# saghen/frizbee

Hardware: AMD Instinct MI355X
Metric: haystacks scored/sec (whole node) + achieved HBM GB/s, 6-char needle vs 10M len-32 haystacks (higher is better)
Workload: dtype u8; 1 GPU; needle 'deadbe' (6 chars) vs 10,000,000 x 32-byte ASCII haystacks per GPU, max_typos=0, mix 5% full / 20% partial / 75% none, seed 12345 (BASELINE.json configs[1]); haystacks_per_gpu=10000000, haystack_len=32, max_typos=0, emulated_reference_backend=AVX-512 (prefilter 64 lanes, Smith-Waterman 64 x u8), ranks_seen=1, backend=none (single process), filter_survivors=499537

## Files before the change

### frizbee_amd/__init__.py

```python
import ctypes as C
import weakref
import enum
import os
from copy import deepcopy
from dataclasses import dataclass, field, replace

import numpy as np

_HERE = os.path.dirname(os.path.abspath(__file__))
_LIB_PATH = os.environ.get("FRIZBEE_HIP_LIB", os.path.join(_HERE, "libfrizbee_hip.so"))

MATCH_DTYPE = np.dtype([("index", "<u4"), ("score", "<u2"), ("exact", "u1"), ("_pad", "u1")])
MATCH_INDICES_DTYPE = np.dtype([("index", "<u4"), ("score", "<u2"), ("exact", "u1"), ("_pad", "u1"), ("positions_begin", "<u4"), ("positions_len", "<u4")])


class FrizbeeError(RuntimeError):
    def __init__(self, code, msg):
        super().__init__(msg)
        self.code = code


class PanicError(FrizbeeError):
    """The reference would `panic!` here; the message is the reference's panic text."""

# ... 47 lines not shown
    max_typos: "int | None" = 0
    casing: CaseMatching = CaseMatching.Smart
    unicode: UnicodeMatching = UnicodeMatching.Smart
    sort: SortStrategy = SortStrategy.ScoreThenIndexAsc
    scoring: Scoring = field(default_factory=Scoring)
    pf_lanes: int = 0
    sw_lanes: int = 0
    matching: Matching = Matching.Fuzzy


class _CScoring(C.Structure):
    _fields_ = [(n, C.c_uint16) for n in ("match_score", "mismatch_penalty", "gap_open_penalty", "gap_extend_penalty", "prefix_bonus",
                                          "capitalization_bonus", "matching_case_bonus", "exact_match_bonus", "delimiter_bonus")]


class _CConfig(C.Structure):
    _fields_ = [("max_typos", C.c_int32), ("casing", C.c_int32), ("unicode", C.c_int32), ("sort", C.c_int32), ("scoring", _CScoring),
                ("pf_lanes", C.c_uint16), ("sw_lanes", C.c_uint16), ("matching", C.c_int32)]


class _CPattern(C.Structure):
    _fields_ = [("needle_utf8", C.c_void_p), ("needle_len", C.c_size_t), ("negated", C.c_int32), ("has_max_typos", C.c_int32), ("max_typos", C.c_int32),
                ("casing", C.c_int32), ("unicode", C.c_int32), ("has_scoring", C.c_int32), ("scoring", _CScoring), ("matching", C.c_int32)]


_lib = None

SYMBOLS = [
    "fzb_last_error", "fzb_config_default", "fzb_matcher_create", "fzb_matcher_clone", "fzb_matcher_free", "fzb_matcher_info", "fzb_matcher_set_pattern", "fzb_matcher_set_config",
    "fzb_corpus_upload", "fzb_corpus_from_device", "fzb_corpus_set_max_len", "fzb_corpus_set_uniform_len", "fzb_corpus_free", "fzb_corpus_len", "fzb_match_list", "fzb_match_list_into",
    "fzb_match_list_device", "fzb_match_list_sorted_device", "fzb_match_list_parallel", "fzb_matches_free", "fzb_radix_sort_matches", "fzb_k_merge_matches",
    "fzb_matcher_reserve", "fzb_debug_unicode_dfa_accepts", "fzb_set_profiling", "fzb_last_timings", "fzb_last_stage_timings", "fzb_last_counters",
    "fzb_multi_matcher_create", "fzb_multi_matcher_free", "fzb_multi_matcher_len", "fzb_multi_match_list", "fzb_multi_match_list_device",
    "fzb_parse_query", "fzb_patterns_free", "fzb_match_list_indices", "fzb_match_indices_free", "fzb_multi_match_list_indices",
    "fzb_match_list_indices_into", "fzb_multi_match_list_into", "fzb_multi_match_list_indices_into",
    "fzb_device_count", "fzb_shard_ranges", "fzb_corpus_upload_sharded", "fzb_sharded_corpus_free", "fzb_sharded_corpus_len", "fzb_sharded_corpus_shards",
    "fzb_sharded_corpus_shard", "fzb_match_list_parallel_sharded", "fzb_debug_lcs_dfa_accepts", "fzb_debug_cdfa_state",
    "fzb_merge_shard_runs", "fzb_corpus_build_view", "fzb_debug_reload_knobs", "fzb_matcher_shard_report",
    "fzb_rccl_unique_id", "fzb_shard_comm_create", "fzb_shard_comm_free", "fzb_shard_comm_rank", "fzb_shard_comm_world", "fzb_match_list_parallel_rccl",
    "fzb_shard_comm_last_exchange",
    "fzb_multi_matcher_set_patterns", "fzb_multi_matcher_set_config", "fzb_multi_matcher_reserve", "fzb_multi_matcher_clone", "fzb_multi_match_list_parallel",
    "fzb_multi_match_list_parallel_sharded", "fzb_multi_match_list_parallel_rccl", "fzb_multi_matcher_shard_report", "fzb_debug_device_allocs",
    "fzb_match_list_top", "fzb_match_list_top_device", "fzb_multi_match_list_top", "fzb_match_list_top_sharded", "fzb_multi_match_list_top_sharded",
    "fzb_corpus_reserve", "fzb_corpus_append", "fzb_corpus_truncate", "fzb_corpus_info", "fzb_debug_corpus_read",
    "fzb_corpus_remove", "fzb_corpus_remove_device", "fzb_corpus_replace", "fzb_corpus_edit_info",
    "fzb_match_list_top_indices", "fzb_match_list_top_indices_device", "fzb_matcher_reserve_top_indices", "fzb_multi_match_list_top_indices",
    "fzb_multi_match_list_top_indices_device", "fzb_multi_match_list_top_indices_fused", "fzb_multi_matcher_reserve_top_indices",
    "fzb_corpus_signature_info", "fzb_debug_needle_signature", "fzb_debug_signature_threshold", "fzb_debug_set_filter_grid",
    "fzb_corpus_set_bias", "fzb_corpus_update_bias", "fzb_corpus_clear_bias", "fzb_corpus_bias_info",
    "fzb_corpus_set_tags", "fzb_corpus_update_tags", "fzb_corpus_clear_tags", "fzb_corpus_set_scope", "fzb_corpus_scope_info",
    "fzb_corpus_generation", "fzb_subset_create", "fzb_subset_free", "fzb_subset_set_indices", "fzb_subset_from_scope", "fzb_subset_info", "fzb_subset_read",
    "fzb_match_list_subset", "fzb_match_list_top_subset", "fzb_match_list_top_subset_device", "fzb_match_list_top_indices_subset",
    "fzb_multi_match_list_subset", "fzb_multi_match_list_top_subset", "fzb_multi_match_list_top_subset_device", "fzb_multi_match_list_top_indices_subset",
    "fzb_debug_set_items_dfa_min", "fzb_debug_set_fused_capture", "fzb_debug_launch_grids", "fzb_corpus_signature_planes_info",
    "fzb_prompt_list_device", "fzb_prompt_top_device",
    "fzb_facets_create", "fzb_facets_free", "fzb_facets_read", "fzb_facets_device", "fzb_matcher_set_facets", "fzb_multi_matcher_set_facets",
    "fzb_match_list_top_sections", "fzb_match_list_top_sections_device", "fzb_multi_match_list_top_sections", "fzb_multi_match_list_top_sections_device",
]


def lib():
    global _lib
    if _lib is None:
        if not os.path.exists(_LIB_PATH):
            raise FrizbeeError(4, f"{_LIB_PATH} is missing: build it with `python -c 'import __graft_entry__ as g; g.build()'` (make -C frizbee_amd/csrc)")
        l = C.CDLL(_LIB_PATH)
        l.fzb_last_error.restype = C.c_char_p
        l.fzb_config_default.argtypes = [C.POINTER(_CConfig)]
        l.fzb_matcher_create.argtypes = [C.POINTER(_CConfig), C.c_char_p, C.c_size_t, C.POINTER(C.c_void_p)]
        l.fzb_matcher_clone.argtypes = [C.c_void_p, C.POINTER(C.c_void_p)]
        l.fzb_matcher_free.argtypes = [C.c_void_p]
        l.fzb_matcher_set_pattern.argtypes = [C.c_void_p, C.c_char_p, C.c_size_t]
        l.fzb_matcher_set_config.argtypes = [C.c_void_p, C.POINTER(_CConfig)]
        l.fzb_matcher_info.argtypes = [C.c_void_p, C.POINTER(C.c_int32)]
        l.fzb_corpus_upload.argtypes = [C.c_void_p, C.c_void_p, C.c_size_t, C.POINTER(C.c_void_p)]
        l.fzb_corpus_from_device.argtypes = [C.c_void_p, C.c_void_p, C.c_int, C.c_size_t, C.c_uint64, C.POINTER(C.c_void_p)]
        l.fzb_corpus_set_max_len.argtypes = [C.c_void_p, C.c_uint32]
        l.fzb_corpus_set_uniform_len.argtypes = [C.c_void_p, C.c_uint32]
        l.fzb_corpus_free.argtypes = [C.c_void_p]
        l.fzb_corpus_len.argtypes = [C.c_void_p]
        l.fzb_corpus_len.restype = C.c_size_t
        l.fzb_match_list.argtypes = [C.c_void_p, C.c_void_p, C.POINTER(C.c_void_p), C.POINTER(C.c_size_t)]
        l.fzb_match_list_into.argtypes = [C.c_void_p, C.c_void_p, C.c_size_t, C.c_size_t, C.c_uint32, C.POINTER(C.c_void_p), C.POINTER(C.c_size_t)]
        l.fzb_match_list_device.argtypes = [C.c_void_p, C.c_void_p, C.c_size_t, C.c_size_t, C.c_uint32, C.c_void_p, C.c_size_t, C.c_void_p, C.c_void_p]
        l.fzb_match_list_sorted_device.argtypes = [C.c_void_p, C.c_void_p, C.c_void_p, C.c_size_t, C.c_void_p, C.c_void_p]
        l.fzb_match_list_parallel.argtypes = [C.c_void_p, C.c_void_p, C.c_size_t, C.POINTER(C.c_void_p), C.POINTER(C.c_size_t)]
        l.fzb_matches_free.argtypes = [C.c_void_p]
        l.fzb_radix_sort_matches.argtypes = [C.c_void_p, C.c_size_t]
        l.fzb_k_merge_matches.argtypes = [C.c_int32, C.c_void_p, C.c_void_p, C.c_size_t, C.c_void_p]
        l.fzb_matcher_reserve.argtypes = [C.c_void_p, C.c_void_p]
        l.fzb_debug_unicode_dfa_accepts.argtypes = [C.c_void_p, C.c_char_p, C.c_size_t]
        l.fzb_set_profiling.argtypes = [C.c_void_p, C.c_int]
        l.fzb_last_timings.argtypes = [C.c_void_p, C.POINTER(C.c_float)]
        l.fzb_last_stage_timings.argtypes = [C.c_void_p, C.POINTER(C.c_float)]
        l.fzb_last_counters.argtypes = [C.c_void_p, C.POINTER(C.c_uint32)]
        l.fzb_multi_matcher_create.argtypes = [C.POINTER(_CConfig), C.POINTER(_CPattern), C.c_size_t, C.POINTER(C.c_void_p)]
        l.fzb_multi_matcher_free.argtypes = [C.c_void_p]
        l.fzb_parse_query.argtypes = [C.c_char_p, C.c_size_t, C.POINTER(C.POINTER(_CPattern)), C.POINTER(C.c_size_t)]
        l.fzb_patterns_free.argtypes = [C.POINTER(_CPattern), C.c_size_t]
        l.fzb_multi_matcher_len.argtypes = [C.c_void_p]
        l.fzb_multi_matcher_len.restype = C.c_size_t
        l.fzb_multi_match_list.argtypes = [C.c_void_p, C.c_void_p, C.POINTER(C.c_void_p), C.POINTER(C.c_size_t)]
        l.fzb_multi_match_list_device.argtypes = [C.c_void_p, C.c_void_p, C.c_size_t, C.c_size_t, C.c_uint32, C.c_void_p, C.c_size_t, C.c_void_p, C.c_void_p]
        l.fzb_match_list_indices.argtypes = [C.c_void_p, C.c_void_p, C.c_void_p, C.c_size_t, C.POINTER(C.c_void_p), C.POINTER(C.c_size_t), C.POINTER(C.c_void_p)]
        l.fzb_match_indices_free.argtypes = [C.c_void_p, C.c_void_p]
        l.fzb_multi_match_list_indices.argtypes = l.fzb_match_list_indices.argtypes
        l.fzb_match_list_indices_into.argtypes = [C.c_void_p, C.c_void_p, C.c_void_p, C.c_size_t, C.c_uint32, C.POINTER(C.c_void_p), C.POINTER(C.c_size_t), C.POINTER(C.c_void_p)]
# ... 4 lines not shown
        l.fzb_corpus_upload_sharded.argtypes = [C.c_void_p, C.c_void_p, C.c_size_t, C.c_int, C.c_int, C.POINTER(C.c_void_p)]
        l.fzb_sharded_corpus_free.argtypes = [C.c_void_p]
        l.fzb_sharded_corpus_len.argtypes = [C.c_void_p]
        l.fzb_sharded_corpus_len.restype = C.c_size_t
        l.fzb_sharded_corpus_shards.argtypes = [C.c_void_p]
        l.fzb_sharded_corpus_shard.argtypes = [C.c_void_p, C.c_int, C.POINTER(C.c_uint64), C.POINTER(C.c_uint64), C.POINTER(C.c_int)]
        l.fzb_match_list_parallel_sharded.argtypes = [C.c_void_p, C.c_void_p, C.POINTER(C.c_void_p), C.POINTER(C.c_size_t)]
        l.fzb_matcher_shard_report.argtypes = [C.c_void_p]
        l.fzb_matcher_shard_report.restype = C.c_char_p
        l.fzb_merge_shard_runs.argtypes = [C.c_void_p, C.c_void_p, C.c_void_p, C.c_void_p, C.c_size_t, C.c_void_p, C.POINTER(C.c_void_p), C.POINTER(C.c_size_t)]
        l.fzb_corpus_build_view.argtypes = [C.c_void_p, C.POINTER(C.c_int)]
        l.fzb_rccl_unique_id.argtypes = [C.c_void_p]
        l.fzb_shard_comm_create.argtypes = [C.c_void_p, C.c_int, C.c_int, C.POINTER(C.c_void_p)]
        l.fzb_shard_comm_free.argtypes = [C.c_void_p]
        l.fzb_shard_comm_rank.argtypes = [C.c_void_p]
        l.fzb_shard_comm_world.argtypes = [C.c_void_p]
        l.fzb_match_list_parallel_rccl.argtypes = [C.c_void_p, C.c_void_p, C.c_uint32, C.c_void_p, C.c_int, C.POINTER(C.c_void_p), C.POINTER(C.c_size_t)]
        l.fzb_shard_comm_last_exchange.argtypes = [C.c_void_p, C.POINTER(C.c_uint64)]
        l.fzb_debug_lcs_dfa_accepts.argtypes = [C.c_void_p, C.c_char_p, C.c_size_t, C.POINTER(C.c_int32)]
        l.fzb_debug_cdfa_state.argtypes = [C.c_void_p, C.c_char_p, C.c_size_t, C.POINTER(C.c_int32)]
        l.fzb_multi_matcher_set_patterns.argtypes = [C.c_void_p, C.POINTER(_CPattern), C.c_size_t]
        l.fzb_multi_matcher_set_config.argtypes = [C.c_void_p, C.POINTER(_CConfig)]
        l.fzb_multi_matcher_reserve.argtypes = [C.c_void_p, C.c_void_p]
        l.fzb_multi_matcher_clone.argtypes = [C.c_void_p, C.POINTER(C.c_void_p)]
        l.fzb_multi_match_list_parallel.argtypes = l.fzb_match_list_parallel.argtypes
        l.fzb_multi_match_list_parallel_sharded.argtypes = l.fzb_match_list_parallel_sharded.argtypes
        l.fzb_multi_match_list_parallel_rccl.argtypes = l.fzb_match_list_parallel_rccl.argtypes
        l.fzb_multi_matcher_shard_report.argtypes = [C.c_void_p]
        l.fzb_multi_matcher_shard_report.restype = C.c_char_p
        l.fzb_debug_device_allocs.argtypes = [C.POINTER(C.c_uint64)]
        l.fzb_match_list_top.argtypes = [C.c_void_p, C.c_void_p, C.c_size_t, C.POINTER(C.c_void_p), C.POINTER(C.c_size_t), C.POINTER(C.c_uint64)]
        l.fzb_match_list_top_device.argtypes = [C.c_void_p, C.c_void_p, C.c_size_t, C.c_void_p, C.c_size_t, C.c_void_p, C.c_void_p]
        l.fzb_multi_match_list_top.argtypes = l.fzb_match_list_top.argtypes
        l.fzb_match_list_top_sharded.argtypes = l.fzb_match_list_top.argtypes
        l.fzb_multi_match_list_top_sharded.argtypes = l.fzb_match_list_top.argtypes
        l.fzb_corpus_reserve.argtypes = [C.c_void_p, C.c_size_t, C.c_uint64]
        l.fzb_corpus_append.argtypes = [C.c_void_p, C.c_void_p, C.c_void_p, C.c_size_t]
        l.fzb_corpus_truncate.argtypes = [C.c_void_p, C.c_size_t]
        l.fzb_corpus_info.argtypes = [C.c_void_p, C.POINTER(C.c_uint64)]
        l.fzb_debug_corpus_read.argtypes = [C.c_void_p, C.c_int, C.c_void_p, C.c_size_t, C.POINTER(C.c_size_t)]
        l.fzb_corpus_remove.argtypes = [C.c_void_p, C.c_void_p, C.c_size_t]
        l.fzb_corpus_remove_device.argtypes = [C.c_void_p, C.c_void_p, C.c_size_t, C.c_void_p, C.c_size_t]
        l.fzb_corpus_replace.argtypes = [C.c_void_p, C.c_void_p, C.c_size_t, C.c_void_p, C.c_void_p]
        l.fzb_corpus_edit_info.argtypes = [C.c_void_p, C.POINTER(C.c_uint64)]
        l.fzb_match_list_top_indices.argtypes = [C.c_void_p, C.c_void_p, C.c_size_t, C.POINTER(C.c_void_p), C.POINTER(C.c_size_t), C.POINTER(C.c_void_p), C.POINTER(C.c_uint64)]
        l.fzb_match_list_top_indices_device.argtypes = [C.c_void_p, C.c_void_p, C.c_size_t, C.c_void_p, C.c_size_t, C.c_void_p, C.c_size_t, C.c_void_p, C.c_void_p]
        l.fzb_matcher_reserve_top_indices.argtypes = [C.c_void_p, C.c_void_p, C.c_size_t, C.c_size_t]
        l.fzb_multi_match_list_top_indices.argtypes = l.fzb_match_list_top_indices.argtypes
        l.fzb_multi_match_list_top_indices_fused.argtypes = l.fzb_match_list_top_indices.argtypes
        l.fzb_multi_match_list_top_indices_device.argtypes = l.fzb_match_list_top_indices_device.argtypes
        l.fzb_multi_matcher_reserve_top_indices.argtypes = l.fzb_matcher_reserve_top_indices.argtypes
        l.fzb_corpus_signature_info.argtypes = [C.c_void_p, C.POINTER(C.c_int), C.POINTER(C.c_uint64)]
        l.fzb_corpus_signature_planes_info.argtypes = l.fzb_corpus_signature_info.argtypes
        l.fzb_debug_needle_signature.argtypes = [C.c_void_p, C.POINTER(C.c_uint32), C.POINTER(C.c_int)]
        l.fzb_debug_signature_threshold.argtypes = []
        l.fzb_debug_signature_threshold.restype = C.c_uint32
        l.fzb_debug_set_filter_grid.argtypes = [C.c_int]
        l.fzb_debug_set_filter_grid.restype = None
        l.fzb_corpus_set_bias.argtypes = [C.c_void_p, C.c_void_p, C.c_size_t]
        l.fzb_corpus_update_bias.argtypes = [C.c_void_p, C.c_void_p, C.c_void_p, C.c_size_t]
        l.fzb_corpus_clear_bias.argtypes = [C.c_void_p]
        l.fzb_corpus_bias_info.argtypes = [C.c_void_p, C.POINTER(C.c_uint64)]
        l.fzb_corpus_set_tags.argtypes = [C.c_void_p, C.c_void_p, C.c_size_t]
        l.fzb_corpus_update_tags.argtypes = [C.c_void_p, C.c_void_p, C.c_void_p, C.c_size_t]
        l.fzb_corpus_clear_tags.argtypes = [C.c_void_p]
        l.fzb_corpus_set_scope.argtypes = [C.c_void_p, C.c_uint16, C.c_uint16]
        l.fzb_corpus_scope_info.argtypes = [C.c_void_p, C.POINTER(C.c_uint64)]
        l.fzb_debug_set_items_dfa_min.argtypes = [C.c_uint32]
        l.fzb_debug_set_items_dfa_min.restype = None
        l.fzb_debug_set_fused_capture.argtypes = [C.c_int]
        l.fzb_debug_set_fused_capture.restype = None
        l.fzb_debug_launch_grids.argtypes = [C.c_char_p, C.c_size_t, C.POINTER(C.c_size_t), C.c_int]
        l.fzb_corpus_generation.argtypes = [C.c_void_p, C.POINTER(C.c_uint64)]
        l.fzb_subset_create.argtypes = [C.c_void_p, C.POINTER(C.c_void_p)]
        l.fzb_subset_free.argtypes = [C.c_void_p]
        l.fzb_subset_free.restype = None
        l.fzb_subset_set_indices.argtypes = [C.c_void_p, C.c_void_p, C.c_size_t]
        l.fzb_subset_from_scope.argtypes = [C.c_void_p, C.c_void_p, C.c_uint16, C.c_uint16]
        l.fzb_subset_info.argtypes = [C.c_void_p, C.POINTER(C.c_uint64)]
        l.fzb_subset_read.argtypes = [C.c_void_p, C.c_void_p, C.c_size_t, C.POINTER(C.c_size_t)]
        l.fzb_match_list_subset.argtypes = [C.c_void_p, C.c_void_p, C.c_void_p, C.c_void_p, C.POINTER(C.c_void_p), C.POINTER(C.c_size_t)]
        l.fzb_match_list_top_subset.argtypes = [C.c_void_p, C.c_void_p, C.c_void_p, C.c_void_p, C.c_size_t, C.POINTER(C.c_void_p), C.POINTER(C.c_size_t), C.POINTER(C.c_uint64)]
        l.fzb_match_list_top_subset_device.argtypes = [C.c_void_p, C.c_void_p, C.c_void_p, C.c_void_p, C.c_size_t, C.c_void_p, C.c_size_t, C.c_void_p, C.c_void_p]
        l.fzb_multi_match_list_subset.argtypes = l.fzb_match_list_subset.argtypes
        l.fzb_multi_match_list_top_subset.argtypes = l.fzb_match_list_top_subset.argtypes
        l.fzb_multi_match_list_top_subset_device.argtypes = l.fzb_match_list_top_subset_device.argtypes
        l.fzb_prompt_list_device.argtypes = [C.c_void_p, C.c_void_p, C.c_void_p, C.c_size_t, C.c_size_t, C.c_uint32, C.c_void_p, C.c_size_t, C.c_void_p, C.c_void_p]
        l.fzb_prompt_top_device.argtypes = [C.c_void_p, C.c_void_p, C.c_void_p, C.c_size_t, C.c_void_p, C.c_size_t, C.c_void_p, C.c_void_p]
        l.fzb_match_list_top_indices_subset.argtypes = [C.c_void_p, C.c_void_p, C.c_void_p, C.c_void_p, C.c_size_t, C.POINTER(C.c_void_p), C.POINTER(C.c_size_t), C.POINTER(C.c_void_p),
                                                        C.POINTER(C.c_uint64)]
        l.fzb_multi_match_list_top_indices_subset.argtypes = l.fzb_match_list_top_indices_subset.argtypes
        l.fzb_facets_create.argtypes = [C.c_void_p, C.POINTER(C.c_void_p)]
        l.fzb_facets_free.argtypes = [C.c_void_p]
        l.fzb_facets_free.restype = None
        l.fzb_facets_read.argtypes = [C.c_void_p, C.POINTER(C.c_uint32)]
        l.fzb_facets_device.argtypes = [C.c_void_p]
        l.fzb_facets_device.restype = C.c_void_p
        l.fzb_matcher_set_facets.argtypes = [C.c_void_p, C.c_void_p]
        l.fzb_multi_matcher_set_facets.argtypes = [C.c_void_p, C.c_void_p]
        l.fzb_match_list_top_sections.argtypes = [C.c_void_p, C.c_void_p, C.c_void_p, C.c_size_t, C.c_size_t, C.c_void_p, C.c_void_p, C.POINTER(C.c_void_p), C.POINTER(C.c_size_t),
                                                  C.POINTER(C.c_uint64)]
        l.fzb_match_list_top_sections_device.argtypes = [C.c_void_p, C.c_void_p, C.c_void_p, C.c_size_t, C.c_size_t, C.c_void_p, C.c_void_p, C.c_void_p, C.c_size_t, C.c_void_p, C.c_void_p]
        l.fzb_multi_match_list_top_sections.argtypes = l.fzb_match_list_top_sections.argtypes
        l.fzb_multi_match_list_top_sections_device.argtypes = l.fzb_match_list_top_sections_device.argtypes
        _lib = l
    return _lib
# ... 85 lines not shown
        self.h = C.c_void_p()
        self._keep = keep
        _check(lib().fzb_corpus_from_device(dev_bytes_ptr, dev_ends_ptr, int(ends_are_u64), n, total_bytes, C.byref(self.h)))
        if uniform_len:
            _check(lib().fzb_corpus_set_uniform_len(self.h, uniform_len))
        if max_len:
            _check(lib().fzb_corpus_set_max_len(self.h, max_len))
        return self

    def build_view(self):
        built = C.c_int()
        _check(lib().fzb_corpus_build_view(self.h, C.byref(built)))
        return bool(built.value)

    def append(self, haystacks=None, *, packed=None):
        data, ends = packed if packed is not None else pack(haystacks)
        data = np.ascontiguousarray(data, dtype=np.uint8)
        ends = np.ascontiguousarray(ends, dtype=np.uint64)
        _check(lib().fzb_corpus_append(self.h, data.ctypes.data, ends.ctypes.data if len(ends) else None, len(ends)))

    def reserve(self, items, nbytes):
        _check(lib().fzb_corpus_reserve(self.h, items, nbytes))

    def truncate(self, n):
        _check(lib().fzb_corpus_truncate(self.h, n))

    def remove(self, indices):
        ix = np.ascontiguousarray(indices, dtype=np.uint32)
        _check(lib().fzb_corpus_remove(self.h, ix.ctypes.data if len(ix) else None, len(ix)))

    def remove_device(self, ptr, stride, count_ptr, max_count):
        _check(lib().fzb_corpus_remove_device(self.h, ptr, stride, count_ptr, max_count))

    def replace(self, indices, haystacks=None, *, packed=None):
        ix = np.ascontiguousarray(indices, dtype=np.uint32)
        data, ends = packed if packed is not None else pack(haystacks)
        data = np.ascontiguousarray(data, dtype=np.uint8)
        ends = np.ascontiguousarray(ends, dtype=np.uint64)
        if len(ix) != len(ends):
            raise FrizbeeError(1, f"Corpus.replace: {len(ix)} indices for {len(ends)} haystacks")
        _check(lib().fzb_corpus_replace(self.h, ix.ctypes.data if len(ix) else None, len(ix), data.ctypes.data, ends.ctypes.data if len(ends) else None))

    EDIT_INFO_FIELDS = ("first", "bytes_written", "view_tiles", "temp_bytes")

    def edit_info(self):
        out = (C.c_uint64 * 4)()
        _check(lib().fzb_corpus_edit_info(self.h, out))
        return dict(zip(self.EDIT_INFO_FIELDS, (int(v) for v in out)))

    INFO_FIELDS = ("items", "item_capacity", "bytes", "byte_capacity", "max_len", "uniform_len", "has_view", "view_nv", "outliers", "ends_u64", "regrows",
                   "h2d_bytes")
    DEBUG_ARRAYS = {"bytes": (0, np.uint8), "ends": (1, None), "vbytes": (2, np.uint8), "vgofs": (3, np.uint32), "vgnv": (4, np.uint8), "vlen": (5, np.uint16),
                    "vperm": (6, np.uint16), "vlong": (7, np.uint32), "sig": (8, np.uint32), "bias": (9, np.int16), "tags": (10, np.uint16),
                    "sig_planes": (11, np.uint64)}

    def set_bias(self, values):
        if values is None:
            _check(lib().fzb_corpus_clear_bias(self.h))
            return
        v = np.asarray(values)
        if v.size and (v.min() < -32768 or v.max() > 32767):
            raise FrizbeeError(1, "Corpus.set_bias: a bias is a signed 16-bit value")
        v = np.ascontiguousarray(v, dtype=np.int16)
        _check(lib().fzb_corpus_set_bias(self.h, v.ctypes.data if len(v) else None, len(v)))

    def _update_column(self, fn, who, indices, v):
        ix = np.ascontiguousarray(indices, dtype=np.uint32)
        if len(ix) != len(v):
            raise FrizbeeError(1, f"{who}: {len(ix)} indices for {len(v)} values")
        _check(fn(self.h, ix.ctypes.data if len(ix) else None, v.ctypes.data if len(v) else None, len(ix)))

    def update_bias(self, indices, values):
        v = np.asarray(values)
        if v.size and (v.min() < -32768 or v.max() > 32767):
            raise FrizbeeError(1, "Corpus.update_bias: a bias is a signed 16-bit value")
        self._update_column(lib().fzb_corpus_update_bias, "Corpus.update_bias", indices, np.ascontiguousarray(v, dtype=np.int16))

    BIAS_INFO_FIELDS = ("has_bias", "capacity", "bias_hi", "device_bytes")

    def bias_info(self):
        out = (C.c_uint64 * 4)()
        _check(lib().fzb_corpus_bias_info(self.h, out))
        return dict(zip(self.BIAS_INFO_FIELDS, (int(x) for x in out)))

    @staticmethod
    def _tags16(values, who):
        v = np.asarray(values)
        if v.size and (v.dtype.kind not in "iub" or v.min() < 0 or v.max() > 65535):
            raise FrizbeeError(1, f"{who}: tags are 16 caller-defined bits (0 .. 65535)")
        return np.ascontiguousarray(v, dtype=np.uint16)

    def set_tags(self, values):
        v = self._tags16(values, "Corpus.set_tags")
        _check(lib().fzb_corpus_set_tags(self.h, v.ctypes.data if len(v) else None, len(v)))

    def update_tags(self, indices, values):
        ix = np.asarray(indices)
        if ix.size and (ix.min() < 0 or ix.max() > 0xFFFFFFFF):
            raise FrizbeeError(1, "Corpus.update_tags: an index is an unsigned 32-bit value")
        self._update_column(lib().fzb_corpus_update_tags, "Corpus.update_tags", ix, self._tags16(values, "Corpus.update_tags"))

    def clear_tags(self):
        _check(lib().fzb_corpus_clear_tags(self.h))

    def set_scope(self, require=0, exclude=0):
        for name, v in (("require", require), ("exclude", exclude)):
            if not 0 <= int(v) <= 65535:
                raise FrizbeeError(1, f"Corpus.set_scope: {name} is a 16-bit mask (0 .. 65535)")
        _check(lib().fzb_corpus_set_scope(self.h, int(require), int(exclude)))

    SCOPE_INFO_FIELDS = ("active", "capacity", "scope", "device_bytes")

    def scope_info(self):
        out = (C.c_uint64 * 4)()
        _check(lib().fzb_corpus_scope_info(self.h, out))
        d = dict(zip(self.SCOPE_INFO_FIELDS, (int(x) for x in out)))
        d["require"], d["exclude"] = d["scope"] & 0xFFFF, d["scope"] >> 16
        return d

    def signature_info(self):
        built, nbytes = C.c_int(), C.c_uint64()
        _check(lib().fzb_corpus_signature_info(self.h, C.byref(built), C.byref(nbytes)))
        return bool(built.value), int(nbytes.value)

    def signature_planes_info(self):
        built, nbytes = C.c_int(), C.c_uint64()
        _check(lib().fzb_corpus_signature_planes_info(self.h, C.byref(built), C.byref(nbytes)))
        return bool(built.value), int(nbytes.value)

    def info(self):
        out = (C.c_uint64 * 12)()
        _check(lib().fzb_corpus_info(self.h, out))
        return dict(zip(self.INFO_FIELDS, (int(v) for v in out)))

    def debug_read(self, what):
        code, dtype = self.DEBUG_ARRAYS[what]
        if dtype is None:
            dtype = np.uint64 if self.info()["ends_u64"] else np.uint32
        n = C.c_size_t()
        rc = lib().fzb_debug_corpus_read(self.h, code, None, 0, C.byref(n))
        if rc != 5:
            _check(rc)
        buf = np.zeros(n.value, np.uint8)
        if n.value:
            _check(lib().fzb_debug_corpus_read(self.h, code, buf.ctypes.data, buf.nbytes, C.byref(n)))
        return buf.view(dtype)

    def generation(self):
        out = C.c_uint64()
        _check(lib().fzb_corpus_generation(self.h, C.byref(out)))
        return out.value

    def __len__(self):
        return lib().fzb_corpus_len(self.h)

    def __del__(self):
        try:
            if getattr(self, "h", None):
                lib().fzb_corpus_free(self.h)
                self.h = None
        except Exception:
            pass


SHARD_BY_COUNT, SHARD_BY_BYTES, SHARD_OVERSUBSCRIBE = 0, 1, 2


class Subset:

    def __init__(self, corpus):
        self.corpus = corpus
        self.h = C.c_void_p()
        _check(lib().fzb_subset_create(corpus.h, C.byref(self.h)))

    def set_indices(self, indices):
        a = np.asarray(indices)
        if a.size and (a.dtype.kind not in "iu" or int(a.min()) < 0 or int(a.max()) > 0xFFFFFFFF):
            raise ValueError("Subset.set_indices: the indices must be integers that fit uint32")
        a = np.ascontiguousarray(a, dtype=np.uint32)
        _check(lib().fzb_subset_set_indices(self.h, a.ctypes.data if len(a) else None, len(a)))
# ... 688 lines not shown
```

### frizbee_amd/csrc/fzb_internal.h

```cpp
#pragma once
#include <stddef.h>
#include <stdint.h>

typedef uint8_t u8;
typedef uint16_t u16;
typedef uint32_t u32;
typedef uint64_t u64;

#define FZB_MAX_ROWS 63
#define FZB_MAX_NEEDLE_BYTES 64
#define FZB_MAX_HAYSTACK_LEN 1024
#define FZB_UNICODE_FWD_CAP 4096u
#define FZB_TILE 1024

struct NeedleDev {
    int32_t rows;
    int32_t nbytes;
    int32_t max_typos;
    int32_t min_haystack_len;
    int32_t unicode;
    int32_t lane_mask;
    u16 match_plus_mismatch;
    u16 mismatch;
    u16 gex;
    u16 gopm;
    u16 prefix, capitalization, matching_case, exact_bonus, delimiter;
    u16 match_score, gap_open;
    u16 _pad;
    alignas(4) u8 raw[FZB_MAX_NEEDLE_BYTES];
    alignas(4) u8 c[FZB_MAX_NEEDLE_BYTES];
    alignas(4) u8 f[FZB_MAX_NEEDLE_BYTES];
    u8 uc[FZB_MAX_ROWS + 1][4];
    u8 uf[FZB_MAX_ROWS + 1][4];
    u8 ulen[FZB_MAX_ROWS + 1];
    static constexpr bool kLong = false;
};

struct NeedleLongDev {
    int32_t rows, nbytes, max_typos, min_haystack_len, unicode, lane_mask;
    u16 match_plus_mismatch, mismatch, gex, gopm;
    u16 prefix, capitalization, matching_case, exact_bonus, delimiter;
    u16 match_score, gap_open, _pad;
    const u8* raw;
    const u8* c;
    const u8* f;
    const u8 (*uc)[4];
    const u8 (*uf)[4];
    const u8* ulen;
    static constexpr bool kLong = true;
};

struct CorpusDev {
    const u8* bytes;
    const void* ends;
    u64 n;
    u64 total_bytes;
    int ends_u64;
    u32 max_len;
    u32 uniform_len;
    const u8* vbytes;
    const u32* vgofs;
    const u8* vgnv;
    const u16* vlen;
    const u16* vperm;
    u32 view_nv;
    const u32* vlong;
    u32 n_long;
    const u32* sig;
    const u64* sig_planes;
};

struct fzb_match_rec {
    u32 index;
    u16 score;
    u8 exact;
    u8 valid;
};

struct fzb_indices_rec {
    u32 index;
    u16 score;
    u8 exact;
    u8 _pad;
    u32 positions_begin;
    u32 positions_len;
};

struct SortBuffers {
    fzb_match_rec* tmp;
    u32* hist;
    size_t cap;
};

struct Workspace {
    u64* bitmap;
    u32* tile_counts;
    u32* surv_idx;
    u32* win;
    u32* overflow;
    u32* dp_scratch;
    size_t dp_scratch_words;
    SortBuffers sort;
    u64* bitmap2;
    u32* tile_counts2;
    u32* items2;
    u32* win2;
    u32* seg_counts;
    u32* counters;
    u64* bitmap_m;
    u32* tile_counts_m;
    u32* marg_list;
    u64* reject_bits;
    u32* tile_rejects;
    u32* rej_prefix;
    size_t cap_marg;
    u32* cls_win;
    u32* cls_lists;
    size_t cap_cls;
    u64* table;
    u8* dfa;
    u8* uni_dfa;
    u8* lcs_dfa;
// ... 1 lines not shown
    size_t cap_items;
    size_t cap_level2;
    bool tables_stale;
    u8* tables_blob;
    u8* tables_host;
    hipEvent_t tables_ev;
    bool tables_ev_pending;
    u32* trace_cells;
    size_t trace_cells_words;
};

struct LaunchCfg {
    int pf_lanes, sw_lanes;
    int filter_mode;
    int filter_exact;
    int window_mode;
    int bias_ok;
    int pad_ok;
    int cfu_ok;
    int cf_ok;
    int cfm_ok;
    int num_cus;
    u32 dead_byte;
};

#define FZB_MAX_RUNS 64
struct RunSet {
    const fzb_match_rec* run[FZB_MAX_RUNS];
    const u32* count[FZB_MAX_RUNS];
    u32 cap[FZB_MAX_RUNS];
    int n;
};

struct RejectOut {
    u64* bits;
    u32* tile_rejects;
    u32* rej_prefix;
    u32* count;
};

struct SegList {
    u32* list;
    u32* counts;
    u32 nseg, stride;
    u32* total_out;
};

#ifdef __HIPCC__
#include <hip/hip_runtime.h>
void fzb_launch_filter(const CorpusDev& c, u64 first, u32 count, const u64* table, const u8* dfa, u32 dead, int rows, int mode, int need, u32 min_len,
                       u64* bitmap, u32* tile_counts, u32* reset_counters, int grid, hipStream_t st, u64* bitmap_m = nullptr, u32* tile_counts_m = nullptr,
                       u64* reject_bits = nullptr, u32* tile_rejects = nullptr, int nul_safe = 0, int acc_lo = -1, const u8* cdfa = nullptr, u32 cdfa_bytes = 0,
                       int cdfa_K = 0, int cdfa_G = 0, u32 needle_sig = 0, int sig_ok = 0,
                       const SegList* seg = nullptr);
bool fzb_filter_sig_applies(const CorpusDev& c, int mode, u32 needle_sig, int sig_ok);
void fzb_launch_sig_planes(const u32* sig, u64 n, u64 t0, u64* planes, int grid, hipStream_t st);
void fzb_launch_scan_rejects(const u32* tile_rejects, u32 ntiles, const u32* reject_count, u32* rej_prefix, hipStream_t st);
void fzb_launch_init_counters(u32* counters, u32 n0, hipStream_t st);
void fzb_launch_compact1(const u64* bitmap, const u32* counts, u32 n_items, const u32* n_items_ptr, const u32* src, u32* out_idx, u32* total_out, int grid, hipStream_t st,
                         u32* total_out2 = nullptr);
void fzb_launch_filter_items(const CorpusDev& c, u64 first, const u32* items, const u32* n_items_ptr, const u64* table, int rows, int mode, int need, u32 min_len,
                             u64* bitmap, u32* tile_counts, int grid, hipStream_t st, const u8* dfa = nullptr, int exact = 0, u32 needle_sig = 0, int sig_ok = 0, u64 n_hint = 0);
bool fzb_filter_items_dfa_applies(const CorpusDev& c, int mode, int exact, const u8* dfa, int rows, u64 n_hint);
void fzb_launch_compact2(const u64* bitmap, const u32* counts, const u32* n_items_ptr, const u32* in_idx, const u32* in_win, u32* out_idx, u32* out_win, u32* total_out,
                         int grid, hipStream_t st);
void fzb_launch_window(const CorpusDev& c, u64 first, const u32* surv_idx, const u32* n_surv_ptr, const NeedleDev& nd, int pf_lanes,
                       u32* win, u64* bitmap2, u32* tile_counts2, u32* counters, int grid, hipStream_t st, const RejectOut* decide = nullptr, u32 max_items = 0);
void fzb_launch_dp(const CorpusDev& c, u64 first, u32 index_offset, const u32* items, const u32* win, const u32* n_items_ptr, const NeedleDev& nd,
                   int sw_lanes, int mode, int wmode, int pad_ok, fzb_match_rec* out, u32 capacity, u32* dev_count, u32* overflow, u32 qcap, u32* counters, int grid, hipStream_t st,
                   const RejectOut* rejects = nullptr, const SegList* seg = nullptr);
bool fzb_dp_short_applies(const CorpusDev& c, int sw_lanes, int mode);
void fzb_launch_compact1_classify(const CorpusDev& c, u64 first, const u64* bitmap, const u32* tile_counts, u32 n_items, u32* out_idx, u32* total_out, const NeedleDev& nd, int sw_lanes,
                                  int wmode, u32 capacity, u32* dev_count, u32* overflow, u32 qcap, u32* counters, u32* win_out, u32* lists, u32 list_stride, int grid, hipStream_t st,
                                  int split_multi);
void fzb_launch_dp_classes(const CorpusDev& c, u64 first, u32 index_offset, const u32* items, const u32* win_in, const u32* n_items_ptr, const NeedleDev& nd, int sw_lanes,
                           int wmode, fzb_match_rec* out, u32 capacity, u32* dev_count, u32* overflow, u32 qcap, u32* counters, u32* win_out, u32* lists, u32 list_stride,
                           int num_cus, hipStream_t st, int part = 0, int split_multi = 0);
void fzb_launch_classes_all(const CorpusDev& c, u64 first, u32 index_offset, const u32* items, const u32* win, const u32* lists, u32 list_stride, const u32* counters,
                            const NeedleDev& nd, int sw_lanes, fzb_match_rec* out, u32 capacity, u32* scratch, int gm, int gc, hipStream_t st);
void fzb_launch_dp_multi(const CorpusDev& c, u64 first, u32 index_offset, const u32* list, const u32* n_list_ptr, const NeedleDev& nd, int sw_lanes, int mode,
                         fzb_match_rec* out, u32 capacity, u32* scratch, int grid, hipStream_t st);
void fzb_launch_unicode_split_wide(const CorpusDev& c, u64 first, const u32* items, const u32* n_items_ptr, int sw_lanes, u32 capacity, u32* overflow, u32 qcap, u32* counters,
                                   int grid, hipStream_t st);
void fzb_launch_dp_unicode(const CorpusDev& c, u64 first, u32 index_offset, const u32* items, const u32* win, const u32* n_items_ptr, const NeedleDev& nd,
                           int sw_lanes, int wmode, fzb_match_rec* out, u32 capacity, u32* dev_count, u32* overflow, u32 qcap, u32* counters,
                           int grid, hipStream_t st, int tform = 0, int multi_front = 0, int one_round_wgs = 0);
void fzb_launch_dp_unicode_multi(const CorpusDev& c, u64 first, u32 index_offset, const u32* list, const u32* n_list_ptr, const NeedleDev& nd, int sw_lanes,
                                 fzb_match_rec* out, u32 capacity, u32* scratch, int grid, hipStream_t st, u32 only_from = 0, int tform = 0, u32* counters = nullptr,
                                 u32* back_end = nullptr, u32 fwd_cap = 0);
void fzb_launch_sort(fzb_match_rec* buf, fzb_match_rec* tmp, const u32* n_ptr, u32* hist, u32 ntiles_cap, int reverse_first, int by_score, int grid, hipStream_t st, int passes = 2);
void fzb_launch_concat_runs(const RunSet& rs, const u32* base_in, u32* total_out, fzb_match_rec* out, u32 capacity, int grid, u32* cut_flag, hipStream_t st);
hipError_t fzb_launch_topk_select(const fzb_match_rec* in, const u32* in_count, u32 in_cap, u32 limit, int by_score, int desc, int one_pass, fzb_match_rec* out, u32 out_cap,
                            u32* out_count, u32* scratch, u32 ntiles_cap, int grid, hipStream_t st);
void fzb_launch_topk_concat(const RunSet& rs, const u32* base_in, u32* total_out, fzb_match_rec* out, u32 capacity, int grid, hipStream_t st);
struct sections_set;
size_t fzb_sections_scratch_words(size_t n_records);
hipError_t fzb_launch_sections_select(const fzb_match_rec* in, const u32* in_count, u32 in_cap, const uint16_t* tags, u64 n_tags, const sections_set& ss, u32 limit, int by_score,
                                      int desc, int one_pass, fzb_match_rec* out, u32* counts, u32* scratch, u32 ntiles_cap, int grid, hipStream_t st);
void fzb_launch_bias_apply(fzb_match_rec* recs, const u32* count, u32 cap, const int16_t* bias, u64 n_bias, u64 first, u32 index_offset, int grid_max, hipStream_t st);
void fzb_launch_scope_drop(const fzb_match_rec* recs, const u32* count, u32 cap, const uint16_t* tags, u64 n_tags, u64 first, u32 index_offset, u32 require, u32 exclude, u64* bitmap,
                           u32* tile_counts, fzb_match_rec* out, u32 capacity, u32* count_out, int grid_max, hipStream_t st, u32* facets = nullptr);
void fzb_launch_facets_records(const fzb_match_rec* recs, const u32* count, u32 cap, const uint16_t* tags, u64 n_tags, u64 first, u32 index_offset, u32 require, u32 exclude, u32* block,
                               int grid_max, hipStream_t st);
void fzb_launch_facets_column(const u32* items, const u32* n_ptr, u32 n, u32 hint, const uint16_t* tags, u64 n_tags, u64 first, u32 require, u32 exclude, u32* block, int grid_max,
                              hipStream_t st);
void fzb_launch_top_items(const fzb_match_rec* head, const u32* head_count, u32 cap, u32* items, u32* n_items, u32* dev_count, int grid, hipStream_t st);
size_t fzb_indices_pack_tile_words(size_t max_records);
void fzb_launch_indices_pack(const fzb_match_rec* head, const u32* head_count, const fzb_match_rec* traced, const u32* traced_count, const u32* npos, const u32* pos, u32 stride,
                             fzb_indices_rec* out, u32 out_cap, u32* dense, u32 dense_cap, u32* dev_count, u32* tiles, u32 max_records, int grid, hipStream_t st);
// ... 49 lines not shown
```

### frizbee_amd/csrc/host.hip

```cpp
#include <hip/hip_runtime.h>

#include <algorithm>
#include <chrono>
#include <cstdio>
#include <cstdlib>
#include <cstring>
#include <memory>
#include <mutex>
#include <new>
#include <thread>
#include <string>
#include <map>
#include <unordered_map>
#include <vector>

#include "host_internal.h"
#include "sig_filter.h"
#include "score_bias.h"
#include "scope.h"
#include "sections.h"
#include "seg_list.h"

namespace {
#include "unicode_case_table.inc"
// ... 740 lines not shown
    m->needle.assign((const char*)needle_utf8, needle_len);
    m->empty = needle_len == 0;
    const fzb_scoring& sc = config->scoring;
    m->use_u8 = fits_in_u8(needle_len, sc);
    int pf = config->pf_lanes, sw = config->sw_lanes;
    if (pf == 0 && sw == 0) detect_host_lanes(m->use_u8, pf, sw);
    else if (sw == 0) sw = m->use_u8 ? pf : pf / 2;
    if (!(pf == 16 || pf == 32 || pf == 64) || !(sw == 8 || sw == 16 || sw == 32 || sw == 64))
        return fail(FZB_ERR_INVALID, "pf_lanes must be 16/32/64 and sw_lanes 8/16/32/64 (or both 0 = auto)");
    m->lc.pf_lanes = pf;
    m->lc.sw_lanes = sw;
    if (m->empty) return FZB_OK;
    bool any_upper = false, ascii = true;
    for (u32 cp : cps) { any_upper |= is_uppercase(cp); ascii &= cp < 0x80; }
    m->case_sensitive = config->casing == FZB_CASE_RESPECT || (config->casing == FZB_CASE_SMART && any_upper);
    m->unicode = config->unicode == FZB_UNICODE_ALWAYS || (config->unicode == FZB_UNICODE_SMART && !ascii);
    m->rows = (int)(m->unicode ? cps.size() : needle_len);
    if (config->matching < FZB_MATCH_FUZZY || config->matching > FZB_MATCH_SUBSTRING) return fail(FZB_ERR_INVALID, "bad matching mode");
    m->literal_mode = config->matching;
    std::string perr = m->literal_mode ? overflow_guard(sc, needle_len, sadd16(std::max(sc.capitalization_bonus, sc.delimiter_bonus), sc.matching_case_bonus), 0)
                                       : overflow_guard(sc, (size_t)m->rows);
    if (!perr.empty()) return fail(FZB_ERR_PANIC, perr);
    m->long_needle = needle_len > FZB_MAX_NEEDLE_BYTES || m->rows > FZB_MAX_ROWS;
    fill_needle_scalars(m, needle_len, cps.size());
    if (m->long_needle) {
        build_long_needle(m, needle_utf8, needle_len, cps);
        return FZB_OK;
    }
    NeedleDev& nd = m->nd;
    for (size_t i = 0; i < needle_len; i++) {
        nd.raw[i] = nd.c[i] = needle_utf8[i];
        nd.f[i] = flip_ascii_byte(m, needle_utf8[i]);
    }
    for (size_t i = 0; i < cps.size() && cps.size() <= FZB_MAX_ROWS; i++) {
        nd.ulen[i] = (u8)encode_utf8(cps[i], nd.uc[i]);
        encode_utf8(m->case_sensitive ? cps[i] : flip_same_width(cps[i]), nd.uf[i]);
    }
    const int k = config->max_typos;
    LaunchCfg& lc = m->lc;
    if (k < 0 || k >= m->rows) {
        lc.filter_mode = 0; lc.filter_exact = 1; lc.window_mode = 2;
    } else if (!m->unicode && k == 0) {
        lc.filter_mode = 1; lc.filter_exact = 1; lc.window_mode = 1;
    } else {
        lc.filter_mode = k == 0 ? 1 : 2; lc.filter_exact = 0; lc.window_mode = 0;
    }
    build_filter_tables(m);
    build_unicode_dfa(m);
    build_lcs_dfa(m);
    build_cdfa(m);
    set_scorer_forms(m, needle_utf8, needle_len);
    m->sig_eligible = !m->unicode && lc.filter_mode == 1 && lc.filter_exact && needle_sig_eligible(needle_utf8, needle_len, k, m->literal_mode);
    m->needle_sig = m->sig_eligible ? needle_sig(needle_utf8, needle_len) : 0u;
    return FZB_OK;
}

int fzb_matcher_create(const fzb_config* config, const uint8_t* needle_utf8, size_t needle_len, fzb_matcher** out) {
    if (!out) return fail(FZB_ERR_INVALID, "null argument");
    std::unique_ptr<fzb_matcher> mp(new fzb_matcher());
    if (int rc = compile_needle(*mp, config, needle_utf8, needle_len)) return rc;
    *out = mp.release();
    return FZB_OK;
}

static int rebuild_matcher(fzb_matcher* m, const fzb_config* config, const uint8_t* needle_utf8, size_t needle_len) {
    CompiledNeedle fresh;
    int rc = compile_needle(fresh, config, needle_utf8, needle_len);
    if (rc) return rc;
    const int num_cus = m->lc.num_cus;
    static_cast<CompiledNeedle&>(*m) = std::move(fresh);
    m->lc.num_cus = num_cus;
    m->ws.tables_stale = true;
    if (m->long_blob_dev) (void)hipFree(m->long_blob_dev);
    m->long_blob_dev = nullptr;
    memset(m->last_counters, 0, sizeof(m->last_counters));
    if (!m->shard_clones.empty()) {
        fzb_config ccfg = m->config;
        ccfg.pf_lanes = (uint16_t)m->lc.pf_lanes;
        ccfg.sw_lanes = (uint16_t)m->lc.sw_lanes;
        bool ok = true;
        for (fzb_matcher* cm : m->shard_clones) ok = ok && rebuild_matcher(cm, &ccfg, needle_utf8, needle_len) == FZB_OK;
        if (!ok) {
            std::vector<fzb_matcher*> drop;
            drop.swap(m->shard_clones);
            for (fzb_matcher* cm : drop) fzb_matcher_free(cm);
            fzb_clear_error();
        }
    }
    return FZB_OK;
}

int fzb_matcher_set_pattern(fzb_matcher* m, const uint8_t* needle_utf8, size_t needle_len) {
    if (!m || (!needle_utf8 && needle_len)) return fail(FZB_ERR_INVALID, "null argument");
    if (m->needle.size() == needle_len && (needle_len == 0 || memcmp(m->needle.data(), needle_utf8, needle_len) == 0)) return FZB_OK;
    const fzb_config cfg = m->config;
    return rebuild_matcher(m, &cfg, needle_utf8, needle_len);
}

}
static bool same_scoring(const fzb_scoring& a, const fzb_scoring& b) {
    return a.match_score == b.match_score && a.mismatch_penalty == b.mismatch_penalty && a.gap_open_penalty == b.gap_open_penalty && a.gap_extend_penalty == b.gap_extend_penalty &&
           a.prefix_bonus == b.prefix_bonus && a.capitalization_bonus == b.capitalization_bonus && a.matching_case_bonus == b.matching_case_bonus &&
           a.exact_match_bonus == b.exact_match_bonus && a.delimiter_bonus == b.delimiter_bonus;
}
static bool same_config(const fzb_config& a, const fzb_config& b) {
    return a.max_typos == b.max_typos && a.casing == b.casing && a.unicode == b.unicode && a.sort == b.sort && a.pf_lanes == b.pf_lanes && a.sw_lanes == b.sw_lanes &&
// ... 65 lines not shown
    if (!fzb_knobs().verify_promises || !c->dev.n || (!uniform_len && !max_len)) return FZB_OK;
    unsigned long long* d = nullptr;
    int prev_dev = 0, own_dev = 0;
    HIPCHK(hipGetDevice(&prev_dev));
    own_dev = prev_dev;
    hipPointerAttribute_t attr;
    if (hipPointerGetAttributes(&attr, c->dev.ends) == hipSuccess && attr.type == hipMemoryTypeDevice) own_dev = attr.device;
    else (void)hipGetLastError();
    struct DeviceGuard {
        int prev, cur;
        ~DeviceGuard() { if (cur != prev) (void)hipSetDevice(prev); }
    } guard{prev_dev, own_dev};
    if (own_dev != prev_dev) HIPCHK(hipSetDevice(own_dev));
    HIPCHK(hipDeviceSynchronize());
    HIPCHK(dev_alloc((void**)&d, 16));
    const unsigned long long init[2] = {0ull, ~0ull};
    hipError_t e = hipMemcpy(d, init, 16, hipMemcpyHostToDevice);
    if (e == hipSuccess) {
        const int grid = (int)fzb_grid_cap((c->dev.n + 255) / 256, 16);
        if (c->dev.ends_u64) FZB_LAUNCH((k_verify_promise<u64>), dim3(grid), dim3(256), 0, 0, (const u64*)c->dev.ends, c->dev.n, c->dev.total_bytes, uniform_len, max_len, d);
        else FZB_LAUNCH((k_verify_promise<u32>), dim3(grid), dim3(256), 0, 0, (const u32*)c->dev.ends, c->dev.n, c->dev.total_bytes, uniform_len, max_len, d);
        e = hipGetLastError();
    }
    unsigned long long got[2] = {0, 0};
    if (e == hipSuccess) e = hipMemcpy(got, d, 16, hipMemcpyDeviceToHost);
    (void)hipFree(d);
    if (e != hipSuccess) return fail(FZB_ERR_HIP, std::string("verifying the corpus promise: ") + hipGetErrorString(e));
    if (got[0])
        return fail(FZB_ERR_INVALID, std::string(what) + ": the end offsets contradict it for " + std::to_string(got[0]) + " haystack(s), first at index " + std::to_string(got[1]) +
                                         " (checked on the device; FZB_VERIFY_PROMISES=0 skips the check)");
    return FZB_OK;
}
extern "C" {
int fzb_corpus_from_device(const void* dev_bytes, const void* dev_ends, int ends_are_u64, size_t n, uint64_t total_bytes, fzb_corpus** out) {
    if (!out || (n && (!dev_bytes || !dev_ends))) return fail(FZB_ERR_INVALID, "null argument");
    if (((uintptr_t)dev_bytes & 15) != 0) return fail(FZB_ERR_INVALID, "dev_bytes must be 16-byte aligned");
    if (n > 0xFFFFFFFFull) return fail(FZB_ERR_PANIC, "too many items in haystack, will overflow the u32 index: " + std::to_string(n) + " > 4294967295 (index offset: 0)");
    auto c = new fzb_corpus();
    c->dev.bytes = (const u8*)dev_bytes;
    c->dev.ends = dev_ends;
    c->dev.ends_u64 = ends_are_u64 != 0;
    c->dev.n = n;
    c->dev.total_bytes = total_bytes;
    *out = c;
    return FZB_OK;
}

void fzb_corpus_free(fzb_corpus* c) {
    if (!c) return;
    if (c->own_bytes) (void)hipFree(c->own_bytes);
    if (c->own_ends) (void)hipFree(c->own_ends);
    if (c->own_sig) (void)hipFree(c->own_sig);
    if (c->own_planes) (void)hipFree(c->own_planes);
    fzb_column_release(c->bias);
    fzb_column_release(c->tags);
    if (c->pair_stage) (void)hipFree(c->pair_stage);
    for (void* q : c->own_view)
        if (q) (void)hipFree(q);
    for (void* q : {c->stage_raw, c->stage_ends, c->stage_tiles, c->stage_stats})
        if (q) (void)hipFree(q);
    delete c;
}
size_t fzb_corpus_len(const fzb_corpus* c) { return c ? (size_t)c->dev.n : 0; }
int fzb_corpus_set_uniform_len(fzb_corpus* c, uint32_t len) {
    if (!c) return fail(FZB_ERR_INVALID, "null argument");
    if (c->own_bytes) {
        if (len == c->dev.uniform_len) return FZB_OK;
        return fail(FZB_ERR_INVALID, "the corpus was uploaded by fzb_corpus_upload, which detected its lengths itself (uniform length " + std::to_string(c->dev.uniform_len) +
                                         ", 0 = not uniform); the promise can only be made for borrowed device memory");
    }
    if (len && (u64)((len + 15u) & ~15u) * (c->dev.n ? c->dev.n - 1 : 0) + len > c->dev.total_bytes) return fail(FZB_ERR_INVALID, "uniform length does not fit the corpus buffer");
    if (len) {
        const int vrc = verify_promise(c, len, 0, ("a uniform length of " + std::to_string(len) + " bytes was promised").c_str());
        if (vrc) return vrc;
    }
    if (!len && c->dev.uniform_len && c->dev.max_len == c->dev.uniform_len) c->dev.max_len = 0;
    c->dev.uniform_len = len;
    if (len) c->dev.max_len = len;
    return fzb_sig_sync_borrowed(c);
}

int fzb_corpus_set_max_len(fzb_corpus* c, uint32_t max_len) {
    if (!c) return fail(FZB_ERR_INVALID, "null argument");
    if (c->own_bytes) {
        if (max_len == 0 || max_len >= c->dev.max_len) return FZB_OK;
        return fail(FZB_ERR_INVALID, "the corpus was uploaded by fzb_corpus_upload, which measured its longest haystack (" + std::to_string(c->dev.max_len) + " bytes); " +
                                         std::to_string(max_len) + " is not an upper bound");
    }
    if (c->dev.uniform_len) {
        if (max_len == 0 || max_len >= c->dev.uniform_len) return FZB_OK;
        return fail(FZB_ERR_INVALID, "the corpus promises a uniform length of " + std::to_string(c->dev.uniform_len) + " bytes; " + std::to_string(max_len) + " is not an upper bound");
    }
    if (max_len && max_len != c->dev.uniform_len) {
        const int vrc = verify_promise(c, 0, max_len, ("a longest haystack of " + std::to_string(max_len) + " bytes was promised").c_str());
        if (vrc) return vrc;
    }
    c->dev.max_len = max_len;
    return fzb_sig_sync_borrowed(c);
}

}
int fzb_bind_device(fzb_matcher* m) {
    int dev = 0;
    HIPCHK(hipGetDevice(&dev));
    if (m->device >= 0) {
        if (dev != m->device)
// ... 527 lines not shown
static int g_debug_filter_grid = 0;
static bool pipe_seg_applies(const Pipe& p) {
    const fzb_matcher* m = p.m;
    const LaunchCfg& lc = m->lc;
    return !p.items_in && !p.trace && !fzb_knobs().no_seg_list && !m->nd.unicode && m->sig_eligible && lc.filter_mode == 1 && lc.filter_exact && lc.window_mode == 1 && lc.cf_ok &&
           fzb_filter_sig_applies(p.cd, 1, m->needle_sig, 1) && fzb_dp_short_applies(p.cd, lc.sw_lanes, 2);
}
static int pipe_filter_stage(Pipe& p) {
    fzb_matcher* m = p.m;
    Workspace& w = m->ws;
    const LaunchCfg& lc = m->lc;
    const NeedleDev& nd = m->nd;
    u32* cnt_c = w.counters;
    p.n_items_ptr = &cnt_c[0];
    p.wmode = lc.window_mode;
    const int need = nd.rows - (nd.max_typos > 0 ? nd.max_typos : 0);
    int exact_wmode = 0;
    const bool uni_typo_exact = nd.unicode && lc.filter_mode == 2 && m->lcs_scalar && m->lcs_states && lc.bias_ok && !p.trace && !fzb_knobs().typo_exact_window && p.cd.max_len != 0 &&
                                p.cd.max_len <= (u32)lc.pf_lanes;
    if (p.items_in) {
        if (lc.filter_mode == 0) {
            HIPCHK(hipMemcpyAsync(&cnt_c[0], p.n_items_in, 4, hipMemcpyDeviceToDevice, p.st));
            p.items = p.items_in;
        } else {
            fzb_launch_filter_items(p.cd, p.first, p.items_in, p.n_items_in, w.table, nd.rows, lc.filter_mode, need, (u32)nd.min_haystack_len, w.bitmap, w.tile_counts, p.cus * 4, p.st,
                                    nd.unicode ? nullptr : w.dfa, lc.filter_exact, m->needle_sig, m->sig_eligible, p.items_hint);
            FZB_STAGE("filter(items)");
            fzb_launch_compact1(w.bitmap, w.tile_counts, 0, p.n_items_in, p.items_in, w.surv_idx, &cnt_c[0], p.cus * 2, p.st);
            FZB_STAGE("compact1(items)");
            p.items = w.surv_idx;
        }
    } else if (lc.filter_mode == 0) {
    } else if (m->uni_dfa_states && lc.bias_ok && !p.trace) {
        FZB_PEV(2);
        fzb_launch_filter(p.cd, p.first, p.cnt, w.table, w.uni_dfa, lc.dead_byte, m->uni_dfa_states - 1, 1, 0, (u32)nd.min_haystack_len, w.bitmap, w.tile_counts, w.counters, p.cus * 8, p.st, nullptr,
                          nullptr, nullptr, nullptr, lc.pad_ok, -1, m->cdfa_src == 2 ? w.cdfa : nullptr, (u32)m->cdfa.size(), m->cdfa_K, m->cdfa_G);
        FZB_PEV(3);
        FZB_STAGE("filter(unicode dfa)");
        fzb_launch_compact1(w.bitmap, w.tile_counts, p.cnt, nullptr, nullptr, w.surv_idx, &cnt_c[0], p.cus * 4, p.st, &cnt_c[1]);
        FZB_STAGE("compact1");
        p.items = w.surv_idx;
        exact_wmode = 1;
    } else if (pipe_seg_applies(p)) {
        const u32 ntiles = (p.cnt + FZB_TILE - 1) / FZB_TILE;
        u32 grid = std::min<u32>(std::min<u32>((u32)p.cus * 8u, FZB_SEG_MAX), ntiles);
        if (g_debug_filter_grid > 0) grid = std::min<u32>(grid, (u32)g_debug_filter_grid);
        grid = std::max<u32>(grid, 1u);
        const u32 stride = tc_tiles_per_run(ntiles, grid) * FZB_TILE;
        if ((size_t)ntiles * FZB_TILE > w.cap_items) return fail(FZB_ERR_INVALID, "internal: the survivor list does not hold the range rounded up to a tile");
        p.seg = SegList{w.surv_idx, w.seg_counts, grid, stride, &cnt_c[0]};
        p.segmented = true;
        FZB_PEV(2);
        fzb_launch_filter(p.cd, p.first, p.cnt, w.table, w.dfa, lc.dead_byte, nd.rows, 1, need, (u32)nd.min_haystack_len, w.bitmap, w.tile_counts, w.counters, (int)grid, p.st, nullptr, nullptr,
                          nullptr, nullptr, lc.pad_ok, -1, nullptr, 0, 0, 0, m->needle_sig, 1, &p.seg);
        FZB_PEV(3);
        FZB_STAGE("filter(lists its survivors)");
        p.items = w.surv_idx;
    } else {
        FZB_PEV(2);
        if (lc.filter_mode == 2 && m->lcs_states)
            fzb_launch_filter(p.cd, p.first, p.cnt, w.table, w.lcs_dfa, lc.dead_byte, m->lcs_states - 1, 1, need, (u32)nd.min_haystack_len, w.bitmap, w.tile_counts, w.counters, p.cus * 8, p.st, nullptr,
                              nullptr, nullptr, nullptr, lc.pad_ok, m->lcs_acc_lo, m->cdfa_src == 3 ? w.cdfa : nullptr, (u32)m->cdfa.size(), m->cdfa_K, m->cdfa_G);
        else
            fzb_launch_filter(p.cd, p.first, p.cnt, w.table, w.dfa, lc.dead_byte, nd.rows, lc.filter_mode, need, (u32)nd.min_haystack_len, w.bitmap, w.tile_counts, w.counters, p.cus * 8, p.st, nullptr, nullptr,
                              nullptr, nullptr, lc.pad_ok, -1, (lc.filter_mode == 1 && m->cdfa_src == 1) ? w.cdfa : nullptr, (u32)m->cdfa.size(), m->cdfa_K, m->cdfa_G, m->needle_sig,
                              m->sig_eligible && lc.filter_mode == 1);
        FZB_PEV(3);
        FZB_STAGE("filter");
        const bool fuse = !nd.unicode && !p.trace && lc.filter_exact && !uni_typo_exact && (p.wmode == 1 || p.wmode == 2) && !fzb_knobs().no_fused_classify && w.cls_win && w.cls_lists &&
                          p.cnt <= (u32)p.cus * 2u * FZB_TILE && ascii_split_classes(m, p.cd);
        if (fuse) {
            fzb_launch_compact1_classify(p.cd, p.first, w.bitmap, w.tile_counts, p.cnt, w.surv_idx, &cnt_c[0], nd, lc.sw_lanes, p.wmode, p.cap32, p.dev_count, w.overflow, pipe_qcap(p), cnt_c,
                                         w.cls_win, w.cls_lists, (u32)w.cap_cls, p.cus * 4, p.st, 1);
            p.classified = true;
            FZB_STAGE("compact1 + classify");
        } else {
            fzb_launch_compact1(w.bitmap, w.tile_counts, p.cnt, nullptr, nullptr, w.surv_idx, &cnt_c[0], p.cus * 4, p.st, uni_typo_exact ? &cnt_c[1] : nullptr);
            FZB_STAGE("compact1");
        }
        p.items = w.surv_idx;
        if (uni_typo_exact) exact_wmode = 3;
    }
    if (exact_wmode) {
        p.wmode = exact_wmode;
    } else if (!lc.filter_exact) {
        fzb_launch_window(p.cd, p.first, p.items, &cnt_c[0], nd, lc.pf_lanes, w.win, w.bitmap2, w.tile_counts2, cnt_c, p.cus * 4, p.st, nullptr, p.items_in ? 0u : p.cnt);
        FZB_STAGE("window");
        fzb_launch_compact2(w.bitmap2, w.tile_counts2, &cnt_c[0], p.items, w.win, w.items2, w.win2, &cnt_c[1], p.cus * 2, p.st);
        FZB_STAGE("compact2");
        p.items = w.items2;
        p.win = w.win2;
        p.n_items_ptr = &cnt_c[1];
        p.wmode = 0;
    }
    return FZB_OK;
}

static bool ascii_split_classes(const fzb_matcher* m, const CorpusDev& cd) {
    const LaunchCfg& lc = m->lc;
    const FzbKnobs& kn = fzb_knobs();
    const bool no_wide = cd.max_len != 0 && cd.max_len <= (u32)lc.sw_lanes;
    const bool classes = lc.cf_ok && !kn.no_dp_classes && !fzb_dp_short_applies(cd, lc.sw_lanes, 2);
    return classes && !no_wide && lc.cfm_ok && !kn.no_dp_cfm;
}
static u32 pipe_qcap(const Pipe& p) { return (u32)std::min<u64>((u64)p.cnt + FZB_UNICODE_FWD_CAP, 0xFFFFFFFFull); }

static int traced_grid(int cus, size_t cnt) { return (int)std::max<size_t>(1, std::min<size_t>((size_t)cus / 2, (cnt + 3) / 4)); }
// ... 2545 lines not shown
```

### frizbee_amd/csrc/host_internal.h

```cpp
#pragma once
#include <hip/hip_runtime.h>

#include <array>
#include <atomic>
#include <functional>
#include <string>
#include <vector>

#include "../../include/frizbee_hip.h"
#include "fzb_internal.h"
#include "indices_union.h"
#include "knobs.h"

int fzb_fail(int code, const std::string& msg);
void fzb_clear_error();
#define HIPCHK(expr)                                                                                            \
    do {                                                                                                        \
        hipError_t e_ = (expr);                                                                                 \
        if (e_ != hipSuccess) return fzb_fail(FZB_ERR_HIP, std::string(#expr) + ": " + hipGetErrorString(e_)); \
    } while (0)

extern std::atomic<uint64_t> g_fzb_dev_allocs;
inline hipError_t fzb_dev_alloc(void** p, size_t bytes) {
    g_fzb_dev_allocs.fetch_add(1, std::memory_order_relaxed);
    return hipMalloc(p, bytes ? bytes : 16);
}

template <typename V>
struct ItemColumn {
    V* data = nullptr;
    u64 cap_items = 0;
    bool live = false;
};
template <typename V>
inline void fzb_column_release(ItemColumn<V>& col) {
    if (col.data) (void)hipFree(col.data);
    col = ItemColumn<V>{};
}

struct fzb_corpus {
    CorpusDev dev{};
    void* own_bytes = nullptr;
    void* own_ends = nullptr;
    void* own_view[6] = {nullptr, nullptr, nullptr, nullptr, nullptr, nullptr};
    u64 cap_items = 0;
    u64 cap_bytes = 0;
    u64 min_len = ~(u64)0;
    u64 max_len = 0;
    u64 n_over256 = 0;
    u64 max_short = 0;
    u64 view_units = 0;
    u64 view_items = 0;
    u64 view_cap_items = 0;
    u64 view_cap_units = 0;
    void* own_sig = nullptr;
    u64 sig_cap_items = 0;
    void* own_planes = nullptr;
    u64 planes_cap_tiles = 0;
    int sig_device = -1;
    ItemColumn<int16_t> bias;
    u32 bias_hi = 0;
    ItemColumn<uint16_t> tags;
    u32 scope_require = 0, scope_exclude = 0;
    void* pair_stage = nullptr;
    u64 pair_stage_cap = 0;
    u64 regrows = 0;
    u64 h2d_bytes = 0;
    u64 edit_info[4] = {0, 0, 0, 0};
    void* stage_raw = nullptr;
    void* stage_ends = nullptr;
    void* stage_tiles = nullptr;
    void* stage_stats = nullptr;
    u64 stage_raw_cap = 0, stage_items_cap = 0, stage_tiles_cap = 0;
    int device = -1;
    u64 generation = 0;
};
inline size_t fzb_corpus_reserved_items(const fzb_corpus* c) { return (size_t)(c->cap_items > c->dev.n ? c->cap_items : c->dev.n); }
inline const int16_t* fzb_corpus_bias(const fzb_corpus* c) { return c->bias.live ? c->bias.data : nullptr; }
inline u32 fzb_corpus_bias_hi(const fzb_corpus* c) { return c->bias.live ? c->bias_hi : 0; }
inline bool fzb_corpus_scoped(const fzb_corpus* c) { return c->tags.data && (c->scope_require | c->scope_exclude) != 0; }

struct fzb_subset {
    const fzb_corpus* corpus = nullptr;
    u64 generation = 0;
    u32* idx = nullptr;
    size_t cap = 0;
    u32* count_dev = nullptr;
    u64* bitmap = nullptr;
    u32* tiles = nullptr;
    bool known = true;
    u64 count = 0;
};

struct fzb_facets {
    const fzb_corpus* corpus = nullptr;
    u32* block = nullptr;
    u32* mirror = nullptr;
    hipEvent_t done = nullptr;
    bool on_event = false;
    bool pending = false;
    int device = -1;
};

template <typename T>
int fzb_dev_renew(T** p, size_t elems) {
    if (*p) HIPCHK(hipFree(*p));
    *p = nullptr;
    HIPCHK(fzb_dev_alloc((void**)p, elems * sizeof(T)));
    return FZB_OK;
}
template <typename T>
// ... 12 lines not shown
    u32* count_host = nullptr;
};
struct OutStaging {
    fzb_match_rec* out_dev = nullptr;
    size_t out_cap = 0;
    u32* count_dev = nullptr;
    FetchHint fetch;
    FetchHint fetch_top;
};
int fzb_out_ensure(OutStaging& o, size_t count);
void fzb_out_release(OutStaging& o);

struct ScopeScratch {
    fzb_match_rec* recs = nullptr;
    size_t recs_cap = 0;
    u64* bitmap = nullptr;
    size_t bitmap_words = 0;
    u32* tiles = nullptr;
    size_t tiles_cap = 0;
    u32* words = nullptr;
    size_t words_cap = 0;
};
int fzb_scope_ensure(ScopeScratch& s, size_t count);
int fzb_scope_ensure_flags(ScopeScratch& s, size_t count);
void fzb_scope_release(ScopeScratch& s);

struct SectionsScratch {
    u32* words = nullptr;
    size_t words_cap = 0;
    u32* stage = nullptr;
    size_t stage_words = 0;
};
int fzb_sections_ensure(SectionsScratch& s, size_t n_records, size_t stage_records);
void fzb_sections_release(SectionsScratch& s);

struct CompiledNeedle {
    fzb_config config{};
    std::string needle;
    bool empty = false, case_sensitive = false, unicode = false, use_u8 = false;
    int literal_mode = 0;
    int rows = 0;
    NeedleDev nd{};
    LaunchCfg lc{};
    std::vector<u64> table;
    std::vector<u8> dfa;
    std::vector<u8> uni_dfa;
    int uni_dfa_states = 0;
    std::vector<u8> lcs_dfa;
    int lcs_states = 0, lcs_acc_lo = 0;
    bool lcs_scalar = false;
    std::vector<u8> cdfa;
    int cdfa_src = 0, cdfa_K = 0, cdfa_G = 0;
    u32 needle_sig = 0;
    bool sig_eligible = false;
    bool long_needle = false;
    bool long_dfa = false;
    bool long_upper = false;
    NeedleLongDev ndl{};
    std::vector<u8> long_blob_host;
    size_t long_off_c = 0, long_off_f = 0, long_off_uc = 0, long_off_uf = 0, long_off_ulen = 0;
};

struct MatcherState : OutStaging {
    Workspace ws{};
    int device = -1;
    bool profiling = false;
    static constexpr int PROF_SLOTS = 32;
    hipEvent_t evring[PROF_SLOTS][5] = {};
    hipStream_t aux_stream = nullptr;
    hipEvent_t ev_fork = nullptr, ev_join = nullptr;
    int ev_filter[PROF_SLOTS] = {};
    u64 prof_calls = 0;

    u32 last_counters[4] = {0, 0, 0, 0};
    u32* trace_sel = nullptr;
    u32* trace_pos = nullptr;
    u32* trace_npos = nullptr;
    size_t trace_cap = 0, trace_pos_words = 0;
    fzb_match_rec* top_head = nullptr;
    fzb_match_rec* top_traced = nullptr;
    u32* top_idx_words = nullptr;
    u32* top_tiles = nullptr;
    size_t top_cap = 0;
    fzb_indices_rec* top_packed = nullptr;
    u32* top_dense = nullptr;
    size_t top_packed_cap = 0, top_dense_words = 0;
    size_t top_last_records = 0, top_last_positions = 0;
    void* long_blob_dev = nullptr;
    u8* long_scratch = nullptr;
    size_t long_scratch_bytes = 0;
    std::vector<fzb_matcher*> shard_clones;
    void* shard_workers = nullptr;
    hipStream_t shard_stream = nullptr;
    hipEvent_t shard_event = nullptr;
    u32* shard_count_host = nullptr;
    int shard_device = -1;
    std::vector<std::array<int, 3>> shard_peers;
    std::string shard_report;
    bool sum_scores = false;
    u32* top_words = nullptr;
    size_t top_words_cap = 0;
    ScopeScratch scope;
    SectionsScratch sections;
    fzb_facets* facets = nullptr;
};

// ... 77 lines not shown
```

### frizbee_amd/csrc/host_upload.hip

```cpp
#include <algorithm>
#include <cstdlib>
#include <cstring>
#include <thread>

#include "host_internal.h"
#include "kernels_common.h"
#include "sig_filter.h"
#include "score_bias.h"

namespace {

constexpr int UP_TILE = 1024;
constexpr int UP_THREADS = 256;

struct UpStats {
    u64 total_padded, min_len, max_len, bad, n_long, max_short;
};

__global__ __launch_bounds__(UP_THREADS) void k_up_tiles(const u64* __restrict__ ends, u64 n, u64 ends_base, u64* __restrict__ tile_sums, UpStats* __restrict__ stats) {
    __shared__ u64 s_sum[UP_THREADS / 64];
    __shared__ u64 s_min[UP_THREADS / 64];
    __shared__ u64 s_max[UP_THREADS / 64];
    __shared__ u64 s_short[UP_THREADS / 64];
    __shared__ u32 s_nlong[UP_THREADS / 64];
// ... 520 lines not shown
    c->dev.vgofs = (const u32*)c->own_view[1];
    c->dev.vgnv = (const u8*)c->own_view[2];
    c->dev.vlen = (const u16*)c->own_view[3];
    c->dev.vperm = (const u16*)c->own_view[4];
    c->dev.vlong = (const u32*)c->own_view[5];
    c->dev.view_nv = (u32)((c->max_short + 15) >> 4);
    c->dev.n_long = (u32)vst.bad;
    c->view_units = units;
    c->view_items = n;
    return FZB_OK;
}

hipError_t measure_resident(fzb_corpus* c, u64 n) {
    hipError_t e = ensure_tiles_scratch(c, 1);
    if (e != hipSuccess) return e;
    UpStats st = UP_STATS_INIT;
    if (n) {
        e = hipMemcpy(c->stage_stats, &UP_STATS_INIT, sizeof(UpStats), hipMemcpyHostToDevice);
        if (e != hipSuccess) return e;
        const unsigned grid = fzb_grid_cap((n + UP_THREADS - 1) / UP_THREADS, 8);
        if (c->dev.ends_u64) FZB_LAUNCH((k_up_measure<u64>), dim3(grid), dim3(UP_THREADS), 0, nullptr, (const u64*)c->dev.ends, n, (UpStats*)c->stage_stats);
        else FZB_LAUNCH((k_up_measure<u32>), dim3(grid), dim3(UP_THREADS), 0, nullptr, (const u32*)c->dev.ends, n, (UpStats*)c->stage_stats);
        e = hipMemcpy(&st, c->stage_stats, sizeof(st), hipMemcpyDeviceToHost);
        if (e != hipSuccess) return e;
    }
    c->min_len = st.min_len; c->max_len = st.max_len; c->n_over256 = st.n_long; c->max_short = st.max_short;
    return hipSuccess;
}

template <typename ET>
__global__ __launch_bounds__(UP_THREADS) void k_sig_build(const u8* __restrict__ bytes, const ET* __restrict__ ends, u32 ulen, u64 first, u64 count, u32* __restrict__ sig) {
    const u64 stride = (u64)gridDim.x * UP_THREADS;
    for (u64 k = (u64)blockIdx.x * UP_THREADS + threadIdx.x; k < count; k += stride) {
        u64 hs;
        u32 L;
        haystack_span_u(ends, ulen, first + k, hs, L);
        L = min(L, 32u);
        const uint4* vp = (const uint4*)(bytes + hs);
        uint4 a = make_uint4(0, 0, 0, 0), b = make_uint4(0, 0, 0, 0);
        if (L > 0) a = vp[0];
        if (L > 16) b = vp[1];
        u32 w[8] = {a.x, a.y, a.z, a.w, b.x, b.y, b.z, b.w};
        u32 s = 0;
#pragma unroll
        for (int j = 0; j < 8; j++) {
            const u32 nvb = L > 4u * j ? L - 4u * j : 0u;
            if (nvb < 4) w[j] &= (1u << (8 * nvb)) - 1;
            s |= sig_of_word(w[j]);
        }
        sig[first + k] = s;
    }
}

bool planes_ensure_room(fzb_corpus* c, u64 items, u64 keep_tiles) {
    const u64 tiles = sig_plane_tiles(items);
    if (c->own_planes && c->planes_cap_tiles >= tiles) return true;
    const size_t tile_bytes = 32 * FZB_SIG_PLANE_WORDS * sizeof(u64);
    void* p = nullptr;
    hipError_t e = fzb_dev_alloc(&p, (size_t)tiles * tile_bytes);
    if (e == hipSuccess && keep_tiles && c->own_planes) e = hipMemcpy(p, c->own_planes, (size_t)std::min(keep_tiles, c->planes_cap_tiles) * tile_bytes, hipMemcpyDeviceToDevice);
    if (c->own_planes) (void)hipFree(c->own_planes);
    c->own_planes = nullptr;
    c->planes_cap_tiles = 0;
    if (e != hipSuccess) {
        if (p) (void)hipFree(p);
        (void)hipGetLastError();
        c->dev.sig_planes = nullptr;
        return false;
    }
    c->own_planes = p;
    c->planes_cap_tiles = tiles;
    if (c->dev.sig_planes) c->dev.sig_planes = (const u64*)p;
    return true;
}

}

int fzb_sig_sync(fzb_corpus* c, u64 n_valid) {
    const u64 n = c->dev.n;
    const bool want = !fzb_knobs().no_signature && n && c->dev.max_len != 0 && c->dev.max_len <= 32;
    if (!want) {
        c->dev.sig = nullptr;
        c->dev.sig_planes = nullptr;
        return FZB_OK;
    }
    if (!c->dev.sig) n_valid = 0, c->dev.sig_planes = nullptr;
    n_valid = std::min(n_valid, n);
    const u64 planes_t0 = c->dev.sig_planes ? n_valid / FZB_SIG_PLANE_TILE : 0;
    if (!c->own_sig || c->sig_cap_items < n) {
        const u64 items = std::max<u64>(n, c->cap_items);
        void* p = nullptr;
        hipError_t e = fzb_dev_alloc(&p, (size_t)items * 4);
        if (e == hipSuccess && n_valid) e = hipMemcpy(p, c->own_sig, (size_t)n_valid * 4, hipMemcpyDeviceToDevice);
        if (e != hipSuccess) {
            if (p) (void)hipFree(p);
            (void)hipGetLastError();
            c->dev.sig = nullptr;
            c->dev.sig_planes = nullptr;
            if (e == hipErrorOutOfMemory) return FZB_OK;
            return fzb_fail(FZB_ERR_HIP, std::string("letter signatures: ") + hipGetErrorString(e));
        }
        if (c->own_sig) (void)hipFree(c->own_sig);
        c->own_sig = p;
        c->sig_cap_items = items;
    }
    if (n > n_valid) {
        const u64 cnt = n - n_valid;
        const unsigned grid = fzb_grid_cap((cnt + UP_THREADS - 1) / UP_THREADS, 32);
        if (c->dev.ends_u64) FZB_LAUNCH((k_sig_build<u64>), dim3(grid), dim3(UP_THREADS), 0, nullptr, c->dev.bytes, (const u64*)c->dev.ends, c->dev.uniform_len, n_valid, cnt, (u32*)c->own_sig);
        else FZB_LAUNCH((k_sig_build<u32>), dim3(grid), dim3(UP_THREADS), 0, nullptr, c->dev.bytes, (const u32*)c->dev.ends, c->dev.uniform_len, n_valid, cnt, (u32*)c->own_sig);
    }
    c->dev.sig = (const u32*)c->own_sig;
    if (planes_ensure_room(c, std::max<u64>(n, c->cap_items), planes_t0)) {
        const u64 tiles = sig_plane_tiles(n);
        if (planes_t0 < tiles) fzb_launch_sig_planes(c->dev.sig, n, planes_t0, (u64*)c->own_planes, (int)fzb_grid_cap(tiles - planes_t0, 8), nullptr);
        c->dev.sig_planes = (const u64*)c->own_planes;
    }
    return FZB_OK;
}

int fzb_sig_sync_borrowed(fzb_corpus* c) {
    int prev_dev = 0, own_dev = 0;
    HIPCHK(hipGetDevice(&prev_dev));
    own_dev = prev_dev;
    hipPointerAttribute_t attr;
    if (c->dev.bytes && hipPointerGetAttributes(&attr, c->dev.bytes) == hipSuccess && attr.type == hipMemoryTypeDevice) own_dev = attr.device;
    else (void)hipGetLastError();
    struct DeviceGuard {
        int prev, cur;
        ~DeviceGuard() { if (cur != prev) (void)hipSetDevice(prev); }
    } guard{prev_dev, own_dev};
    if (own_dev != prev_dev) HIPCHK(hipSetDevice(own_dev));
    if (c->own_sig && c->sig_device != own_dev) {
        (void)hipFree(c->own_sig);
        c->own_sig = nullptr; c->sig_cap_items = 0;
        if (c->own_planes) (void)hipFree(c->own_planes);
        c->own_planes = nullptr; c->planes_cap_tiles = 0;
    }
    c->dev.sig = nullptr;
    c->dev.sig_planes = nullptr;
    if (!fzb_knobs().verify_promises) return FZB_OK;
    HIPCHK(hipDeviceSynchronize());
    const int rc = fzb_sig_sync(c, 0);
    if (rc) return rc;
    if (c->dev.sig) {
        c->sig_device = own_dev;
        HIPCHK(hipDeviceSynchronize());
        HIPCHK(hipGetLastError());
    }
    return FZB_OK;
}

int fzb_build_filter_view(fzb_corpus* c) {
    if (!c->dev.n || c->dev.uniform_len || c->dev.vbytes) return FZB_OK;
    if (!c->own_bytes) {
        const hipError_t e = measure_resident(c, c->dev.n);
        if (e != hipSuccess) return fzb_fail(FZB_ERR_HIP, std::string("filter view: ") + hipGetErrorString(e));
    }
    return view_sync(c, 0);
}

extern "C" int fzb_corpus_build_view(fzb_corpus* c, int* out_built) {
    if (!c) return fzb_fail(FZB_ERR_INVALID, "null argument");
    const int rc = fzb_build_filter_view(c);
    if (out_built) *out_built = c->dev.vbytes != nullptr;
    return rc;
}

int fzb_corpus_upload_impl(const uint8_t* bytes, const uint64_t* end_offsets, size_t n, uint64_t ends_base, fzb_corpus** out) {
    if (!out || (n && (!bytes || !end_offsets))) return fzb_fail(FZB_ERR_INVALID, "null argument");
    if (n > 0xFFFFFFFFull)
        return fzb_fail(FZB_ERR_PANIC, "too many items in haystack, will overflow the u32 index: " + std::to_string(n) + " > 4294967295 (index offset: 0)");
    if (n && end_offsets[n - 1] < ends_base) return fzb_fail(FZB_ERR_INVALID, "end_offsets must be non-decreasing");
    int device = 0;
    HIPCHK(hipGetDevice(&device));
    const u64 raw_bytes = n ? end_offsets[n - 1] - ends_base : 0;
    const u64 ntiles = up_tiles(n);
    auto c = new fzb_corpus();
    c->device = device;
    u8* d_raw = nullptr;
    u64* d_ends64 = nullptr;
    auto cleanup = [&]() {
        for (void* p : {(void*)d_raw, (void*)d_ends64})
            if (p) (void)hipFree(p);
    };
    auto bail = [&](hipError_t e, const char* what) {
        cleanup();
        fzb_corpus_free(c);
        return fzb_fail(FZB_ERR_HIP, std::string("corpus upload (") + what + "): " + hipGetErrorString(e));
    };
    hipError_t e = fzb_dev_alloc((void**)&d_raw, raw_bytes + 96);
    if (e == hipSuccess) e = fzb_dev_alloc((void**)&d_ends64, std::max<size_t>(n, 1) * 8);
    if (e == hipSuccess) e = ensure_tiles_scratch(c, ntiles);
// ... 338 lines not shown
        tags_made(c, 0);
        if (e != hipSuccess) return fzb_fail(FZB_ERR_HIP, std::string("fzb_corpus_set_scope: ") + hipGetErrorString(e));
        HIPCHK(hipDeviceSynchronize());
    }
    c->scope_require = require;
    c->scope_exclude = exclude;
    return FZB_OK;
}

int fzb_corpus_scope_info(const fzb_corpus* c, uint64_t out[4]) {
    if (!c || !out) return fzb_fail(FZB_ERR_INVALID, "null argument");
    out[0] = fzb_corpus_scoped(c) ? 1 : 0;
    out[1] = c->tags.cap_items;
    out[2] = (u64)c->scope_require | ((u64)c->scope_exclude << 16);
    out[3] = c->tags.cap_items * sizeof(uint16_t);
    return FZB_OK;
}

int fzb_corpus_reserve(fzb_corpus* c, size_t items, uint64_t bytes) {
    int rc = grow_begin(c, "fzb_corpus_reserve");
    if (rc) return rc;
    if (items > 0xFFFFFFFFull)
        return fzb_fail(FZB_ERR_PANIC, "too many items in haystack, will overflow the u32 index: " + std::to_string(items) + " > 4294967295 (index offset: 0)");
    if (!c->dev.ends_u64 && bytes + 96 > 0xFFFFFFF0ull)
        return fzb_fail(FZB_ERR_CAPACITY, "fzb_corpus_reserve: a corpus whose end offsets are 32-bit holds less than 4 GiB of padded bytes");
    const u64 regrows = c->regrows;
    hipError_t e = canon_ensure_room(c, items, bytes + 96, false);
    c->regrows = regrows;
    if (e == hipSuccess) e = stage_ensure_room(c, c->cap_items - c->dev.n, c->cap_bytes - c->dev.total_bytes);
    if (e == hipSuccess) e = ensure_tiles_scratch(c, up_tiles(c->cap_items) + 1);
    if (e == hipSuccess) e = col_follow(c, c->bias, c->cap_items);
    if (e == hipSuccess) e = col_follow(c, c->tags, c->cap_items);
    if (e != hipSuccess) return fzb_fail(FZB_ERR_HIP, std::string("fzb_corpus_reserve: ") + hipGetErrorString(e));
    if (!fzb_knobs().no_filter_view) {
        const u64 live_units = c->dev.vbytes ? c->view_units : 0;
        e = view_ensure_room(c, c->cap_items, std::max(c->view_cap_units, view_units_bound(c->cap_items, c->cap_bytes)), c->view_items, live_units);
        if (e == hipErrorOutOfMemory) (void)hipGetLastError();
        else if (e != hipSuccess) return fzb_fail(FZB_ERR_HIP, std::string("fzb_corpus_reserve (filter view): ") + hipGetErrorString(e));
    }
    if (!fzb_knobs().no_signature && (!c->dev.n || (c->dev.max_len != 0 && c->dev.max_len <= 32)) && c->sig_cap_items < c->cap_items) {
        void* p = nullptr;
        e = fzb_dev_alloc(&p, (size_t)c->cap_items * 4);
        if (e == hipSuccess && c->dev.sig && c->dev.n) e = hipMemcpy(p, c->own_sig, (size_t)c->dev.n * 4, hipMemcpyDeviceToDevice);
        if (e == hipSuccess) {
            if (c->own_sig) (void)hipFree(c->own_sig);
            c->own_sig = p;
            c->sig_cap_items = c->cap_items;
            if (c->dev.sig) c->dev.sig = (const u32*)p;
        } else {
            if (p) (void)hipFree(p);
            (void)hipGetLastError();
        }
    }
    if (!fzb_knobs().no_signature && (!c->dev.n || (c->dev.max_len != 0 && c->dev.max_len <= 32)) && c->own_sig && c->sig_cap_items >= c->cap_items)
        (void)planes_ensure_room(c, c->cap_items, c->dev.sig_planes ? sig_plane_tiles(c->dev.n) : 0);
    HIPCHK(hipDeviceSynchronize());
    return FZB_OK;
}

int fzb_corpus_append(fzb_corpus* c, const uint8_t* bytes, const uint64_t* end_offsets, size_t n_new) {
    if (!c || (n_new && !end_offsets)) return fzb_fail(FZB_ERR_INVALID, "null argument");
    const u64 raw = n_new ? end_offsets[n_new - 1] : 0;
    if (raw && !bytes) return fzb_fail(FZB_ERR_INVALID, "null argument");
    int rc = grow_begin(c, "fzb_corpus_append");
    if (rc) return rc;
    if (!n_new) return FZB_OK;
    const u64 n_old = c->dev.n;
    if (n_old + (u64)n_new > 0xFFFFFFFFull)
        return fzb_fail(FZB_ERR_PANIC, "too many items in haystack, will overflow the u32 index: " + std::to_string(n_old + (u64)n_new) + " > 4294967295 (index offset: 0)");
    hipError_t e = stage_ensure_room(c, n_new, raw);
    if (e == hipSuccess) e = h2d_all({H2DJob{c->stage_ends, end_offsets, n_new * 8}, H2DJob{c->stage_raw, bytes, (size_t)raw}}, c->device);
    UpStats st = UP_STATS_INIT;
    if (e == hipSuccess) e = batch_measure((const u64*)c->stage_ends, n_new, 0, (u64*)c->stage_tiles, (UpStats*)c->stage_stats, &st);
    if (e != hipSuccess) return fzb_fail(FZB_ERR_HIP, std::string("fzb_corpus_append (host to device): ") + hipGetErrorString(e));
    if (st.bad) return fzb_fail(FZB_ERR_INVALID, "end_offsets must be non-decreasing");
    const u64 used = c->dev.total_bytes - 96;
    const u64 total = used + st.total_padded + 96;
    if (!c->dev.ends_u64 && total > 0xFFFFFFF0ull)
        return fzb_fail(FZB_ERR_CAPACITY, "fzb_corpus_append: the batch takes the padded list to 4 GiB, beyond this corpus' 32-bit end offsets; upload such a list in one piece");
    e = canon_ensure_room(c, n_old + n_new, total, true);
    if (e == hipSuccess) e = col_follow(c, c->bias, std::max<u64>(n_old + n_new, c->cap_items));
    if (e == hipSuccess) e = col_follow(c, c->tags, std::max<u64>(n_old + n_new, c->cap_items));
    if (e != hipSuccess) return fzb_fail(FZB_ERR_HIP, std::string("fzb_corpus_append (room for the batch): ") + hipGetErrorString(e));
    batch_lay_out((const u8*)c->stage_raw, (const u64*)c->stage_ends, n_new, 0, (const u64*)c->stage_tiles, (u8*)c->own_bytes, used, c->own_ends, n_old, c->dev.ends_u64 != 0, true);
    c->h2d_bytes += raw + (u64)n_new * 8;
    c->dev.n = n_old + n_new;
    c->dev.total_bytes = total;
    c->generation++;
    c->min_len = std::min(c->min_len, st.min_len);
    c->max_len = std::max(c->max_len, st.max_len);
    c->max_short = std::max(c->max_short, st.max_short);
    c->n_over256 += st.n_long;
    set_measured(c);
    rc = view_sync(c, n_old);
    if (!rc) rc = fzb_sig_sync(c, n_old);
    e = hipDeviceSynchronize();
    if (e == hipSuccess) e = hipGetLastError();
    if (rc) return rc;
    if (e != hipSuccess) return fzb_fail(FZB_ERR_HIP, std::string("fzb_corpus_append (layout kernels): ") + hipGetErrorString(e));
    return FZB_OK;
}

int fzb_corpus_truncate(fzb_corpus* c, size_t n) {
    int rc = grow_begin(c, "fzb_corpus_truncate");
    if (rc) return rc;
    if (n > c->dev.n) return fzb_fail(FZB_ERR_INVALID, "fzb_corpus_truncate: " + std::to_string(n) + " is beyond the corpus' " + std::to_string(c->dev.n) + " haystacks");
    if (n == c->dev.n) return FZB_OK;
    u64 used = 0;
// ... 4 lines not shown
        used = (last + 15) & ~(u64)15;
    }
    const u64 old_used = c->dev.total_bytes - 96;
    if (old_used > used) HIPCHK(hipMemsetAsync((u8*)c->own_bytes + used, 0, old_used - used, nullptr));
    hipError_t e = measure_resident(c, n);
    if (e == hipSuccess) e = col_truncate(c->bias, c->dev.n, n);
    if (e == hipSuccess) e = col_truncate(c->tags, c->dev.n, n);
    if (e != hipSuccess) return fzb_fail(FZB_ERR_HIP, std::string("fzb_corpus_truncate: ") + hipGetErrorString(e));
    c->dev.n = n;
    c->dev.total_bytes = used + 96;
    c->generation++;
    set_measured(c);
    rc = view_sync(c, n);
    if (!rc) rc = fzb_sig_sync(c, n);
    e = hipDeviceSynchronize();
    if (e == hipSuccess) e = hipGetLastError();
    if (rc) return rc;
    if (e != hipSuccess) return fzb_fail(FZB_ERR_HIP, std::string("fzb_corpus_truncate: ") + hipGetErrorString(e));
    return FZB_OK;
}

int fzb_corpus_info(const fzb_corpus* c, uint64_t out[12]) {
    if (!c || !out) return fzb_fail(FZB_ERR_INVALID, "null argument");
    const bool own = c->own_bytes != nullptr;
    out[0] = c->dev.n;
    out[1] = own ? std::max<u64>(c->cap_items, c->dev.n) : c->dev.n;
    out[2] = c->dev.total_bytes >= 96 && own ? c->dev.total_bytes - 96 : c->dev.total_bytes;
    out[3] = own ? c->cap_bytes - 96 : c->dev.total_bytes;
    out[4] = c->dev.max_len;
    out[5] = c->dev.uniform_len;
    out[6] = c->dev.vbytes != nullptr;
    out[7] = c->dev.vbytes ? c->dev.view_nv : 0;
    out[8] = c->dev.vbytes ? c->dev.n_long : 0;
    out[9] = c->dev.ends_u64 != 0;
    out[10] = c->regrows;
    out[11] = c->h2d_bytes;
    return FZB_OK;
}

int fzb_corpus_signature_info(const fzb_corpus* c, int* out_built, uint64_t* out_bytes) {
    if (!c) return fzb_fail(FZB_ERR_INVALID, "null argument");
    if (out_built) *out_built = c->dev.sig != nullptr;
    if (out_bytes) *out_bytes = c->dev.sig ? (uint64_t)c->dev.n * 4 : 0;
    return FZB_OK;
}

int fzb_corpus_signature_planes_info(const fzb_corpus* c, int* out_built, uint64_t* out_bytes) {
    if (!c) return fzb_fail(FZB_ERR_INVALID, "null argument");
    if (out_built) *out_built = c->dev.sig_planes != nullptr;
    if (out_bytes) *out_bytes = c->dev.sig_planes ? sig_plane_words(c->dev.n) * 8 : 0;
    return FZB_OK;
}

int fzb_debug_corpus_read(const fzb_corpus* c, int what, void* host_out, size_t cap_bytes, size_t* out_bytes) {
    if (!c || !out_bytes) return fzb_fail(FZB_ERR_INVALID, "null argument");
    const u64 n = c->dev.n, groups = up_tiles(n) * (UP_TILE / 64);
    const bool view = c->dev.vbytes != nullptr;
    const void* src = nullptr;
    size_t bytes = 0;
    switch (what) {
        case 0: src = c->dev.bytes; bytes = c->own_bytes ? (size_t)c->dev.total_bytes : 0; break;
        case 1: src = c->dev.ends; bytes = (size_t)n * (c->dev.ends_u64 ? 8 : 4); break;
        case 2: src = c->dev.vbytes; bytes = view ? (size_t)c->view_units * 16 : 0; break;
        case 3: src = c->dev.vgofs; bytes = view ? (size_t)groups * 4 : 0; break;
        case 4: src = c->dev.vgnv; bytes = view ? (size_t)groups : 0; break;
        case 5: src = c->dev.vlen; bytes = view ? (size_t)n * 2 : 0; break;
        case 6: src = c->dev.vperm; bytes = view ? (size_t)n * 2 : 0; break;
        case 7: src = c->dev.vlong; bytes = view ? (size_t)c->dev.n_long * 4 : 0; break;
        case 8: src = c->dev.sig; bytes = c->dev.sig ? (size_t)n * 4 : 0; break;
        case 9: src = c->bias.data; bytes = c->bias.live ? (size_t)n * sizeof(int16_t) : 0; break;
        case 10: src = c->tags.data; bytes = c->tags.live ? (size_t)n * sizeof(uint16_t) : 0; break;
        case 11: src = c->dev.sig_planes; bytes = c->dev.sig_planes ? (size_t)sig_plane_words(n) * 8 : 0; break;
        default: return fzb_fail(FZB_ERR_INVALID, "fzb_debug_corpus_read: unknown array " + std::to_string(what));
    }
    *out_bytes = bytes;
    if (!bytes) return FZB_OK;
    if (!host_out || cap_bytes < bytes) return fzb_fail(FZB_ERR_CAPACITY, "fzb_debug_corpus_read: the array has " + std::to_string(bytes) + " bytes");
    HIPCHK(hipDeviceSynchronize());
    HIPCHK(hipMemcpy(host_out, src, bytes, hipMemcpyDeviceToHost));
    return FZB_OK;
}

}

namespace {

struct EdStats {
    u64 bad_pos, first, count, new_bytes, new_items, start0;
    u64 max_chunk_bytes, forward_ok;
};
const EdStats ED_STATS_INIT{~(u64)0, ~(u64)0, 0, 0, 0, 0, 0, 0};

struct EdSrc {
    const u32* bitmap;
    const u32* ridx;
    const u32* rk;
    const u64* bends;
    u32 n_repl;
    u32 replace;
};

__device__ __forceinline__ bool ed_touched(const EdSrc& s, u64 i) { return (s.bitmap[i >> 5] >> (i & 31)) & 1u; }
__device__ __forceinline__ void ed_batch_item(const EdSrc& s, u64 i, u64* from, u64* len) {
    u32 lo = 0, hi = s.n_repl;
    while (hi - lo > 1) {
        const u32 mid = (lo + hi) >> 1;
        if (s.ridx[mid] <= (u32)i) lo = mid;
        else hi = mid;
    }
    const u32 k = s.rk[lo];
    const u64 b = k ? s.bends[k - 1] : 0;
    *from = b;
    *len = s.bends[k] - b;
}

__global__ __launch_bounds__(UP_THREADS) void k_ed_mark(const u32* __restrict__ idx, u64 stride_words, const u32* __restrict__ dev_count, u64 max_count, u64 n,
                                                        u32* __restrict__ bitmap, EdStats* __restrict__ st) {
    const u64 cnt = dev_count ? min((u64)*dev_count, max_count) : max_count;
    u64 first = ~(u64)0, bad = ~(u64)0;
    const u64 stride = (u64)gridDim.x * UP_THREADS;
    for (u64 k = (u64)blockIdx.x * UP_THREADS + threadIdx.x; k < cnt; k += stride) {
        const u32 v = idx[k * stride_words];
        if (v >= n) bad = min(bad, k);
        else {
            atomicOr(&bitmap[v >> 5], 1u << (v & 31));
// ... 460 lines not shown
```

### frizbee_amd/csrc/kernels_filter.hip

```cpp
#include "kernels_common.h"
#include "compact1.h"
#include "dfa_lds.h"
#include "sig_filter.h"
#include "items_filter.h"
#include "seg_list.h"
#include <algorithm>
#include <cstdlib>

template <typename TW, int MODE>
__device__ __forceinline__ void filter_step(TW& st, u32 b, const TW* T) {
    TW t = T[b];
    if (MODE == 1) {
        st += st & t;
    } else {
        TW u = st & t;
        st = (st + u) | (st & ~t);
    }
}

template <typename TW, int MODE>
__device__ __forceinline__ void filter_word(TW& st, u32 w, u32 nbytes, const TW* T) {
    if (nbytes >= 4) {
        filter_step<TW, MODE>(st, w & 0xFF, T);
        filter_step<TW, MODE>(st, (w >> 8) & 0xFF, T);
// ... 152 lines not shown
    dfa_load_lds(dfa, dfa_g, rows);
    const u32 ntiles = (count + FZB_TILE - 1) / FZB_TILE;
    for (u32 tile = blockIdx.x; tile < ntiles; tile += gridDim.x) {
        if (tid == 0) s_cnt = 0;
        __syncthreads();
        const u32 cnt = dfa_stream_tile<ET>(bytes, ends, first, count, tile, tid, ulen, min_len, acc_lo, dfa, bitmap);
        if (lane_id() == 0 && cnt) atomicAdd(&s_cnt, cnt);
        __syncthreads();
        if (tid == 0) tile_counts[tile] = s_cnt;
        __syncthreads();
    }
}

__device__ __forceinline__ uint4 sig_mask_vec(uint4 q, u32 nbytes) {
    u32 w[4] = {q.x, q.y, q.z, q.w};
#pragma unroll
    for (int j = 0; j < 4; j++) {
        const u32 nvb = nbytes > 4u * j ? nbytes - 4u * j : 0u;
        w[j] = nvb >= 4 ? w[j] : (w[j] & ((1u << (8 * nvb)) - 1));
    }
    return make_uint4(w[0], w[1], w[2], w[3]);
}
__device__ __forceinline__ u32 dfa_chain16(u32 st, const uint4& q, const u8* dfa) {
    const u32 w[4] = {q.x, q.y, q.z, q.w};
#pragma unroll
    for (int j = 0; j < 4; j++) {
        st = dfa_step<0>(st, w[j], dfa);
        st = dfa_step<1>(st, w[j], dfa);
        st = dfa_step<2>(st, w[j], dfa);
        st = dfa_step<3>(st, w[j], dfa);
    }
    return st;
}
__device__ __forceinline__ u32 seg_list_tile(const u32* s_bits, u32 t, u32 tile, bool write_words, u64* __restrict__ bitmap, u32* __restrict__ tile_counts, u32* __restrict__ seg_out, u32 seg_n) {
    const u32 l32 = t & 31u;
    const u32 wl = s_bits[l32];
    const u32 c = (u32)__popc(wl);
    u32 incl = tc_scan16(c);
    incl += (l32 & 16u) ? (u32)__builtin_amdgcn_readlane((int)incl, 15) : 0u;
    const u32 excl = incl - c, total = (u32)__builtin_amdgcn_readlane((int)incl, 31);
    if (t == 0) tile_counts[tile] = total;
    if (write_words && t < FZB_TILE / 64) bitmap[(size_t)tile * (FZB_TILE / 64) + t] = (u64)s_bits[2 * t] | ((u64)s_bits[2 * t + 1] << 32);
    if (total) {
#pragma unroll
        for (int p = 0; p < FZB_TILE / 256; p++) {
            const u32 pos = (u32)(p * 256) + t, w = pos >> 5;
            const u32 word = (u32)__builtin_amdgcn_ds_bpermute((int)(w << 2), (int)wl), before = (u32)__builtin_amdgcn_ds_bpermute((int)(w << 2), (int)excl);
            if ((word >> (pos & 31)) & 1) seg_out[tc_rank32(seg_n + before, word, pos & 31)] = tile * FZB_TILE + pos;
        }
    }
    return total;
}

template <typename ET>
__device__ __forceinline__ void sig_planes_run(const u8* __restrict__ bytes, const ET* __restrict__ ends, const u64* __restrict__ planes, u32 nsig, u64 first, u32 count, u32 rows,
                                               u32 min_len, u32 acc_lo, u64* __restrict__ bitmap, u32* __restrict__ tile_counts, u32 ulen, u32 gather_max, const SegList& seg, u8* dfa, const u8* __restrict__ dfa_g) {
    constexpr u32 B = FZB_SIG_BATCH_TILES;
    static_assert(B * 16 <= 256 && B * 32 <= 256 && B * FZB_TILE <= 65536, "a batch's words are one per thread, its positions fit the queue's u16");
    u8* const behind = dfa + FZB_DFA_LDS_BYTES(rows);
    u64* const s_cand = (u64*)behind;
    u32* const s_dec = (u32*)(behind + 128 * B);
    u32* const s_tq = (u32*)(behind + 256 * B);
    u16* const queue = (u16*)(behind + 256 * B + 4 * B);
    const u32 tid = threadIdx.x;
    const u32 ntiles = (count + FZB_TILE - 1) / FZB_TILE;
    const u64 tile0 = first / FZB_TILE;
    u32 t_begin, t_end, seg_n = 0;
    tc_run(ntiles, seg.stride / FZB_TILE, blockIdx.x, &t_begin, &t_end);
    u32* const seg_out = seg.list + (size_t)blockIdx.x * seg.stride;
    const u32 j = tid >> 4, w = tid & 15u;
    auto load_cand = [&](u32 tb, u32 nb) -> u64 {
        if (tid >= nb * 16) return 0;
        u64 cand = sig_plane_valid(tb + j, w, count);
        const u64* pl = planes + sig_plane_index(tile0 + tb + j, 0, w);
        u32 m = nsig;
        while (m) {
            u64 v[4];
#pragma unroll
            for (int q = 0; q < 4; q++) {
                v[q] = ~0ull;
                if (m) {
                    v[q] = pl[(u32)__builtin_ctz(m) * FZB_SIG_PLANE_WORDS];
                    m &= m - 1u;
                }
            }
            cand &= (v[0] & v[1]) & (v[2] & v[3]);
        }
        return cand;
    };
    u64 cand = t_begin < t_end ? load_cand(t_begin, min(B, t_end - t_begin)) : 0;
    dfa_load_lds(dfa, dfa_g, (int)rows);
    for (u32 tb = t_begin; tb < t_end; tb += B) {
        const u32 nb = min(B, t_end - tb);
        if (tb != t_begin) cand = load_cand(tb, nb);
        if (tid < B * 32) s_dec[tid] = 0;
        const u32 c = (u32)__popcll(cand);
        const u32 incl = tc_scan16(c);
        if (tid < B * 16) {
            s_cand[tid] = cand;
            if (w == 15) s_tq[j] = incl;
        }
        __syncthreads();
        u32 qbase = 0, QT = 0, dense = 0;
#pragma unroll
        for (u32 k = 0; k < B; k++) {
            const u32 q = s_tq[k];
            if (q > gather_max) dense |= 1u << k;
            else {
                if (k < j) qbase += q;
                QT += q;
            }
        }
        if (tid < nb * 16 && !((dense >> j) & 1)) {
            u32 slot = qbase + incl - c;
            for (u64 m = cand; m; m &= m - 1) queue[slot++] = (u16)(j * FZB_TILE + w * 64 + (u32)__builtin_ctzll(m));
        }
        for (u32 d = dense; d; d &= d - 1) {
            const u32 k = (u32)__builtin_ctz(d);
            (void)dfa_stream_tile<ET, true>(bytes, ends, first, count, tb + k, (int)tid, ulen, min_len, acc_lo, dfa, bitmap, s_dec + 32 * k);
        }
        __syncthreads();
        for (u32 e0 = 0; e0 < QT; e0 += 512) {
            const bool two = e0 + 256 < QT;
            u32 pos[2] = {0, 0};
            bool has[2];
            uint4 a[2], b[2];
            u32 L[2];
#pragma unroll
            for (int r = 0; r < 2; r++) {
                const u32 e = e0 + (u32)r * 256 + tid;
                has[r] = e < QT && (r == 0 || two);
                a[r] = make_uint4(0, 0, 0, 0);
                b[r] = make_uint4(0, 0, 0, 0);
                L[r] = 0;
                if (has[r]) {
                    pos[r] = queue[e];
                    u64 hs;
                    haystack_span_u(ends, ulen, first + (u64)tb * FZB_TILE + pos[r], hs, L[r]);
                    const uint4* vp = (const uint4*)(bytes + hs);
                    if (L[r] > 0) a[r] = vp[0];
                    if (L[r] > 16) b[r] = vp[1];
                }
            }
#pragma unroll
            for (int r = 0; r < 2; r++) {
                if (L[r] < 16) a[r] = sig_mask_vec(a[r], L[r]);
                if (L[r] < 32) b[r] = sig_mask_vec(b[r], L[r] > 16 ? L[r] - 16 : 0u);
            }
            u32 st[2] = {0, 0};
            if (two) {
                const u32 w0[8] = {a[0].x, a[0].y, a[0].z, a[0].w, b[0].x, b[0].y, b[0].z, b[0].w}, w1[8] = {a[1].x, a[1].y, a[1].z, a[1].w, b[1].x, b[1].y, b[1].z, b[1].w};
#pragma unroll
                for (int k = 0; k < 8; k++) {
                    st[0] = dfa_step<0>(st[0], w0[k], dfa); st[1] = dfa_step<0>(st[1], w1[k], dfa);
                    st[0] = dfa_step<1>(st[0], w0[k], dfa); st[1] = dfa_step<1>(st[1], w1[k], dfa);
                    st[0] = dfa_step<2>(st[0], w0[k], dfa); st[1] = dfa_step<2>(st[1], w1[k], dfa);
                    st[0] = dfa_step<3>(st[0], w0[k], dfa); st[1] = dfa_step<3>(st[1], w1[k], dfa);
                }
            } else {
                st[0] = dfa_chain16(0u, a[0], dfa);
                st[0] = dfa_chain16(st[0], b[0], dfa);
            }
#pragma unroll
            for (int r = 0; r < 2; r++)
                if (has[r] && L[r] >= min_len && st[r] >= acc_lo) atomicOr(&s_dec[pos[r] >> 5], 1u << (pos[r] & 31));
        }
        __syncthreads();
        for (u32 k = 0; k < nb; k++) {
            u32 t = tid;
            asm volatile("" : "+v"(t));
            seg_n += seg_list_tile(s_dec + 32 * k, t, tb + k, !((dense >> k) & 1), bitmap, tile_counts, seg_out, seg_n);
        }
        __syncthreads();
    }
    if (tid == 0) seg.counts[blockIdx.x] = seg_n;
}

template <typename ET, bool SEG, bool PLANES = false>
__global__ __launch_bounds__(256) __attribute__((amdgpu_waves_per_eu(8, 8))) void k1_dfa_sig(const u8* __restrict__ bytes, const ET* __restrict__ ends, const u32* __restrict__ sig, u32 nsig, u64 first, u32 count,
                                                  const u8* __restrict__ dfa_g, int rows, u32 min_len, u32 acc_lo, u64* __restrict__ bitmap, u32* __restrict__ tile_counts,
                                                  u32* __restrict__ reset_counters, u32 ulen, u32 gather_max, SegList seg) {
    if (blockIdx.x == 0 && threadIdx.x < 16) reset_counters[threadIdx.x] = 0;
    extern __shared__ __attribute__((aligned(16))) u8 dfa[];
    if constexpr (PLANES) {
        static_assert(SEG, "the plane form lists its survivors");
        dfa_require_lds_base0(dfa);
        sig_planes_run<ET>(bytes, ends, (const u64*)sig, nsig, first, count, (u32)rows, min_len, acc_lo, bitmap, tile_counts, ulen, gather_max, seg, dfa, dfa_g);
        return;
    }
    u32& s_cnt = *(u32*)(dfa + FZB_DFA_LDS_BYTES(rows));
    u32& s_q = *(u32*)(dfa + FZB_DFA_LDS_BYTES(rows) + 4);
    u32* const s_bits = (u32*)(dfa + FZB_DFA_LDS_BYTES(rows) + 16);
    u16* const queue = (u16*)(dfa + FZB_DFA_LDS_BYTES(rows) + 16 + 128);
    const int tid = threadIdx.x, lane = tid & 63;
    dfa_require_lds_base0(dfa);
    dfa_load_lds(dfa, dfa_g, rows);
    const u32 ntiles = (count + FZB_TILE - 1) / FZB_TILE;
    const bool vec = (first & 3) == 0;
    auto load_sigs = [&](u32 tile) -> uint4 {
        const u32 li = tile * FZB_TILE + 4u * (u32)tid;
        uint4 s = make_uint4(0, 0, 0, 0);
        if (vec && li + 4 <= count) {
            s = *(const uint4*)(sig + first + li);
        } else {
            if (li < count) s.x = sig[first + li];
            if (li + 1 < count) s.y = sig[first + li + 1];
            if (li + 2 < count) s.z = sig[first + li + 2];
            if (li + 3 < count) s.w = sig[first + li + 3];
        }
        return s;
    };
    u32 t_begin = blockIdx.x, t_end = ntiles, seg_n = 0;
    if (SEG) tc_run(ntiles, seg.stride / FZB_TILE, blockIdx.x, &t_begin, &t_end);
    u32* const seg_out = SEG ? seg.list + (size_t)blockIdx.x * seg.stride : nullptr;
    for (u32 tile = t_begin; tile < t_end; tile += SEG ? 1u : gridDim.x) {
        if (tid == 0) s_cnt = 0, s_q = 0;
        if (tid < 32) s_bits[tid] = 0;
        const uint4 s = load_sigs(tile);
        __syncthreads();
        const u32 sv[4] = {s.x, s.y, s.z, s.w};
        u64 pb[4];
        u32 tot = 0;
#pragma unroll
        for (int j = 0; j < 4; j++) {
            pb[j] = __ballot(sig_passes(sv[j], nsig));
            tot += (u32)__popcll(pb[j]);
        }
        if (tot) {
            u32 base = 0;
            if (lane == 0) base = atomicAdd(&s_q, tot);
            base = __shfl(base, 0);
            const u64 below = ((u64)1 << lane) - 1;
#pragma unroll
            for (int j = 0; j < 4; j++) {
                if ((pb[j] >> lane) & 1) queue[base + (u32)__popcll(pb[j] & below)] = (u16)(4 * tid + j);
                base += (u32)__popcll(pb[j]);
            }
        }
        __syncthreads();
        const u32 Q = s_q;
// ... 546 lines not shown
                }
                const u64 b = __ballot(matched);
                if (lane_id() == 0) {
                    bitmap[(tile * FZB_TILE + p * 256) / 64 + (tid >> 6)] = b;
                    cnt += __popcll(b);
                }
            }
        }
        if (lane_id() == 0 && cnt) atomicAdd(&s_cnt, cnt);
        __syncthreads();
        if (tid == 0) tile_counts[tile] = s_cnt;
        __syncthreads();
    }
}

#define FZB_ITEMS_DFA_MIN_SHORT 100000u
#define FZB_ITEMS_DFA_MIN_RAGGED 0xFFFFFFFFu
static u32 g_items_dfa_min_short = FZB_ITEMS_DFA_MIN_SHORT, g_items_dfa_min_ragged = FZB_ITEMS_DFA_MIN_RAGGED;
extern "C" void fzb_debug_set_items_dfa_min(uint32_t n) {
    g_items_dfa_min_short = n ? n : FZB_ITEMS_DFA_MIN_SHORT;
    g_items_dfa_min_ragged = n ? n : FZB_ITEMS_DFA_MIN_RAGGED;
}
bool fzb_filter_items_dfa_applies(const CorpusDev& c, int mode, int exact, const u8* dfa, int rows, u64 n_hint) {
    const bool shortc = c.max_len != 0 && c.max_len <= 32;
    return mode == 1 && exact && dfa && rows >= 1 && rows <= FZB_MAX_ROWS && !fzb_knobs().no_items_dfa && n_hint != 0 && n_hint >= (u64)(shortc ? g_items_dfa_min_short : g_items_dfa_min_ragged);
}

void fzb_launch_filter_items(const CorpusDev& c, u64 first, const u32* items, const u32* n_items_ptr, const u64* table, int rows, int mode, int need, u32 min_len,
                             u64* bitmap, u32* tile_counts, int grid, hipStream_t st, const u8* dfa, int exact, u32 needle_sig, int sig_ok, u64 n_hint) {
    if (fzb_filter_items_dfa_applies(c, mode, exact, dfa, rows, n_hint)) {
        const size_t lds = (size_t)(rows + 1) * FZB_DFA_STRIDE + 16;
        const bool shortc = c.max_len != 0 && c.max_len <= 32;
        const bool use_sig = shortc && fzb_filter_sig_applies(c, mode, needle_sig, sig_ok);
        const u64 tiles = (n_hint + FZB_TILE - 1) / FZB_TILE;
        const int g = (int)std::max<u64>(1, std::min<u64>((u64)std::max(1, grid) * 2, tiles));
#define FZB_K1ID(ET, SIG, SHORT) FZB_LAUNCH((k1_items_dfa<ET, SIG, SHORT>), dim3(g), dim3(256), lds, st, c.bytes, (const ET*)c.ends, c.sig, needle_sig, first, items, n_items_ptr, dfa, rows, min_len, (u32)rows, bitmap, tile_counts, c.uniform_len)
        if (c.ends_u64) { if (use_sig) FZB_K1ID(u64, true, true); else if (shortc) FZB_K1ID(u64, false, true); else FZB_K1ID(u64, false, false); }
        else            { if (use_sig) FZB_K1ID(u32, true, true); else if (shortc) FZB_K1ID(u32, false, true); else FZB_K1ID(u32, false, false); }
#undef FZB_K1ID
        return;
    }
    const bool w64 = (mode == 1) ? rows > 31 : rows > 32;
#define FZB_K1I(TW, MODE, ET) FZB_LAUNCH((k1_items<TW, MODE, ET>), dim3(grid), dim3(256), 0, st, c.bytes, (const ET*)c.ends, first, items, n_items_ptr, table, rows, need, min_len, bitmap, tile_counts)
    if (c.ends_u64) {
        if (mode == 1) { if (w64) FZB_K1I(u64, 1, u64); else FZB_K1I(u32, 1, u64); }
        else           { if (w64) FZB_K1I(u64, 2, u64); else FZB_K1I(u32, 2, u64); }
    } else {
        if (mode == 1) { if (w64) FZB_K1I(u64, 1, u32); else FZB_K1I(u32, 1, u32); }
        else           { if (w64) FZB_K1I(u64, 2, u32); else FZB_K1I(u32, 2, u32); }
    }
#undef FZB_K1I
}

__global__ __launch_bounds__(256) void k_sig_planes_build(const u32* __restrict__ sig, u64 n, u64 t0, u64* __restrict__ planes) {
    __shared__ u64 s_pl[32 * FZB_SIG_PLANE_WORDS];
    const u32 tid = threadIdx.x, lane = tid & 63, wave = tid >> 6;
    const u64 tiles = sig_plane_tiles(n);
    for (u64 tile = t0 + blockIdx.x; tile < tiles; tile += gridDim.x) {
#pragma unroll
        for (u32 p = 0; p < FZB_TILE / 256; p++) {
            const u64 i = tile * FZB_TILE + p * 256 + tid;
            const u32 s = i < n ? sig[i] : 0u;
            u64 mine = 0;
            for (u32 b = 0; b < 32; b++) {
                const u64 bal = __ballot((s >> b) & 1u);
                if (lane == b) mine = bal;
            }
            if (lane < 32) s_pl[lane * FZB_SIG_PLANE_WORDS + p * 4 + wave] = mine;
        }
        __syncthreads();
        u64* out = planes + sig_plane_index(tile, 0, 0);
        out[tid] = s_pl[tid];
        out[tid + 256] = s_pl[tid + 256];
        __syncthreads();
    }
}
void fzb_launch_sig_planes(const u32* sig, u64 n, u64 t0, u64* planes, int grid, hipStream_t st) {
    FZB_LAUNCH(k_sig_planes_build, dim3(std::max(1, grid)), dim3(256), 0, st, sig, n, t0, planes);
}

bool fzb_filter_sig_applies(const CorpusDev& c, int mode, u32 needle_sig, int sig_ok) {
    return mode == 1 && c.max_len != 0 && c.max_len <= 32 && sig_ok && needle_sig && c.sig && !fzb_knobs().no_signature;
}

void fzb_launch_filter(const CorpusDev& c, u64 first, u32 count, const u64* table, const u8* dfa, u32 dead, int rows, int mode, int need, u32 min_len,
                       u64* bitmap, u32* tile_counts, u32* reset_counters, int grid, hipStream_t st, u64* bitmap_m, u32* tile_counts_m, u64* reject_bits, u32* tile_rejects, int nul_safe,
                       int acc_lo, const u8* cdfa, u32 cdfa_bytes, int cdfa_K, int cdfa_G, u32 needle_sig, int sig_ok, const SegList* seg) {
    const u32 acc = acc_lo < 0 ? (u32)rows : (u32)acc_lo;
    const u32 ntiles = (count + FZB_TILE - 1) / FZB_TILE;
    const int cus = std::max(1, grid / 8);
    if (grid > (int)ntiles) grid = ntiles;
    if (grid < 1) grid = 1;
    if (mode == 1) {
        const size_t lds = (size_t)(rows + 1) * FZB_DFA_STRIDE + 16;
        const bool shortc = c.max_len != 0 && c.max_len <= 32;
        if (fzb_filter_sig_applies(c, mode, needle_sig, sig_ok)) {
            const u32 gmax = std::min<u32>(FZB_SIG_GATHER_MAX, FZB_TILE);
            const bool planes = seg && c.sig_planes && first % FZB_TILE == 0 && !fzb_knobs().no_sig_planes;
            const size_t lds_s = planes ? FZB_DFA_LDS_BYTES(rows) + FZB_SIG_BATCH_TILES * (4 + 256 + 2 * (size_t)gmax) : lds + 128 + 2 * FZB_TILE;
#define FZB_K1S(ET, SEG, PL, G, S) FZB_LAUNCH((k1_dfa_sig<ET, SEG, PL>), dim3(G), dim3(256), lds_s, st, c.bytes, (const ET*)c.ends, PL ? (const u32*)c.sig_planes : c.sig, needle_sig, first, count, dfa, rows, min_len, acc, bitmap, tile_counts, reset_counters, c.uniform_len, gmax, S)
            if (planes) {
                if (g_fzb_record_grids) fzb_record_grid("k1_dfa_sig_planes", seg->nseg);
                if (c.ends_u64) FZB_K1S(u64, true, true, seg->nseg, *seg); else FZB_K1S(u32, true, true, seg->nseg, *seg);
            } else if (seg) {
                if (c.ends_u64) FZB_K1S(u64, true, false, seg->nseg, *seg); else FZB_K1S(u32, true, false, seg->nseg, *seg);
            } else {
                if (c.ends_u64) FZB_K1S(u64, false, false, grid, SegList{}); else FZB_K1S(u32, false, false, grid, SegList{});
            }
#undef FZB_K1S
            return;
        }
        if (shortc) {
#define FZB_K1D(ET) FZB_LAUNCH((k1_dfa<ET>), dim3(grid), dim3(256), lds, st, c.bytes, (const ET*)c.ends, first, count, dfa, rows, min_len, dead, acc, bitmap, tile_counts, reset_counters, c.uniform_len)
            if (c.ends_u64) FZB_K1D(u64); else FZB_K1D(u32);
#undef FZB_K1D
            return;
        }
        const FzbKnobs& kn = fzb_knobs();
        const bool composite = cdfa && !kn.no_cdfa && (cdfa_G == 4 || cdfa_G == 2);
        u32 kg = 1;
        for (int i = 0; i < cdfa_G; i++) kg *= (u32)cdfa_K;
        if (composite && c.vbytes && !kn.no_filter_view && first % FZB_TILE == 0 && (first + count == c.n || count % FZB_TILE == 0) && c.view_nv != 0 && c.view_nv <= 16) {
            const size_t lds_v = ((cdfa_bytes + 15) & ~(size_t)15) + 16 + 128;
            const int g = std::max(1, std::min<int>(cus * 6, (int)ntiles));
            const bool len_free = nul_safe && acc >= 1;
            const bool wide = nul_safe && len_free && ntiles < (u32)cus * 2u;
#define FZB_K1VA const_cast<const u8*>(c.vbytes), c.vgofs, c.vgnv, c.vlen, c.vperm, first, count, cdfa, cdfa_bytes, (u32)cdfa_K, kg, min_len, dead, acc, bitmap, tile_counts, reset_counters
#define FZB_K1V(SAN, G, NV, LEN) FZB_LAUNCH((k1_cdfa_view<SAN, G, NV, LEN>), dim3(g), dim3(256), lds_v, st, FZB_K1VA)
#define FZB_K1W(G, NV) FZB_LAUNCH((k1_cdfa_view<false, G, NV, false, 1024>), dim3(g), dim3(1024), lds_v, st, FZB_K1VA)
#define FZB_K1V_S(SAN, G, NV) do { if (!SAN && wide) FZB_K1W(G, NV); else if (!SAN && len_free) FZB_K1V(SAN, G, NV, false); else FZB_K1V(SAN, G, NV, true); } while (0)
#define FZB_K1V_NV(SAN, G) do { if (c.view_nv <= 8) FZB_K1V_S(SAN, G, 8); else FZB_K1V_S(SAN, G, 16); } while (0)
#define FZB_K1V_G(SAN) do { if (cdfa_G == 4) FZB_K1V_NV(SAN, 4); else FZB_K1V_NV(SAN, 2); } while (0)
            if (nul_safe) FZB_K1V_G(false); else FZB_K1V_G(true);
#undef FZB_K1V_G
#undef FZB_K1V_NV
#undef FZB_K1V_S
#undef FZB_K1W
#undef FZB_K1V
#undef FZB_K1VA
            if (c.n_long) {
                const u32 ns_o = (cdfa_bytes - 256u) / kg;
                const u32 wpw = ((cdfa_bytes + 15) & ~(size_t)15) + (size_t)4 * 64 * ns_o + 16 <= 60 * 1024 ? 4u : 1u;
                const size_t lds_o = ((cdfa_bytes + 15) & ~(size_t)15) + (size_t)wpw * 64 * ns_o + 16;
                const int go = (int)std::max<u32>(1u, std::min<u32>((c.n_long + wpw - 1) / wpw, (u32)cus * 16u));
#define FZB_K1O(ET, SAN, G) FZB_LAUNCH((k1_cdfa_outliers<ET, SAN, G>), dim3(go), dim3(64 * wpw), lds_o, st, c.bytes, (const ET*)c.ends, first, count, c.vlong, c.n_long, cdfa, cdfa_bytes, (u32)cdfa_K, kg, ns_o, min_len, dead, acc, bitmap, tile_counts)
#define FZB_K1O_G(ET, SAN) do { if (cdfa_G == 4) FZB_K1O(ET, SAN, 4); else FZB_K1O(ET, SAN, 2); } while (0)
                if (c.ends_u64) { if (nul_safe) FZB_K1O_G(u64, false); else FZB_K1O_G(u64, true); }
                else            { if (nul_safe) FZB_K1O_G(u32, false); else FZB_K1O_G(u32, true); }
#undef FZB_K1O_G
#undef FZB_K1O
            }
            return;
        }
        if (composite) {
            const size_t lds_c = ((cdfa_bytes + 15) & ~(size_t)15) + 16;
// ... 79 lines not shown
```

### frizbee_amd/csrc/sig_filter.h

```cpp
#pragma once
#include <stddef.h>
#include <stdint.h>

#ifndef FZB_SIG_FN
#define FZB_SIG_FN __host__ __device__ inline
#endif

FZB_SIG_FN uint32_t sig_bit(uint32_t b) {
    const uint32_t l = (b | 0x20u) - 'a';
    return l < 26u ? l : 26u + b % 6u;
}
FZB_SIG_FN uint32_t sig_of_byte(uint32_t b) { return b ? 1u << sig_bit(b) : 0u; }
FZB_SIG_FN uint32_t sig_of_word(uint32_t w) { return sig_of_byte(w & 0xFF) | sig_of_byte((w >> 8) & 0xFF) | sig_of_byte((w >> 16) & 0xFF) | sig_of_byte(w >> 24); }
FZB_SIG_FN uint32_t sig_of_bytes(const uint8_t* p, size_t n) {
    uint32_t s = 0;
    for (size_t i = 0; i < n; i++) s |= sig_of_byte(p[i]);
    return s;
}
FZB_SIG_FN uint32_t needle_sig(const uint8_t* needle, size_t n) { return sig_of_bytes(needle, n); }
FZB_SIG_FN bool sig_passes(uint32_t sig, uint32_t nsig) { return (sig & nsig) == nsig; }

FZB_SIG_FN bool needle_sig_eligible(const uint8_t* needle, size_t n, int max_typos, int literal_mode) {
    if (literal_mode != 0 || max_typos != 0 || n == 0) return false;
    for (size_t i = 0; i < n; i++)
        if (needle[i] == 0 || needle[i] >= 0x80) return false;
    return true;
}

#define FZB_SIG_PLANE_TILE 1024u
#define FZB_SIG_PLANE_WORDS 16u
FZB_SIG_FN uint64_t sig_plane_tiles(uint64_t n_items) { return (n_items + FZB_SIG_PLANE_TILE - 1) / FZB_SIG_PLANE_TILE; }
FZB_SIG_FN uint64_t sig_plane_words(uint64_t n_items) { return sig_plane_tiles(n_items) * 32u * FZB_SIG_PLANE_WORDS; }
FZB_SIG_FN uint64_t sig_plane_index(uint64_t tile, uint32_t bit, uint32_t word) { return (tile * 32u + bit) * FZB_SIG_PLANE_WORDS + word; }
FZB_SIG_FN uint64_t sig_plane_valid(uint64_t tile, uint32_t word, uint64_t count) {
    const uint64_t base = tile * FZB_SIG_PLANE_TILE + 64u * word;
    return base >= count ? 0ull : count - base >= 64u ? ~0ull : (1ull << (count - base)) - 1ull;
}
FZB_SIG_FN void sig_planes_transpose_ref(const uint32_t* sig, uint64_t n, uint64_t* planes) {
    const uint64_t words = sig_plane_words(n);
    for (uint64_t k = 0; k < words; k++) planes[k] = 0;
    for (uint64_t i = 0; i < n; i++)
        for (uint32_t b = 0; b < 32; b++)
            if ((sig[i] >> b) & 1u) planes[sig_plane_index(i / FZB_SIG_PLANE_TILE, b, (uint32_t)(i % FZB_SIG_PLANE_TILE) / 64u)] |= 1ull << (i % 64u);
}
FZB_SIG_FN uint64_t sig_plane_candidates(const uint64_t* planes, uint64_t tile, uint32_t word, uint32_t nsig) {
    uint64_t c = ~0ull;
    for (uint32_t m = nsig; m; m &= m - 1u) c &= planes[sig_plane_index(tile, (uint32_t)__builtin_ctz(m), word)];
    return c;
}
#ifndef FZB_SIG_BATCH_TILES
#define FZB_SIG_BATCH_TILES 8u
#endif

#ifndef FZB_SIG_GATHER_MAX
#define FZB_SIG_GATHER_MAX 384u
#endif
```

### include/frizbee_hip.h

```cpp
#ifndef FRIZBEE_HIP_H
#define FRIZBEE_HIP_H

#include <stddef.h>
#include <stdint.h>

#ifdef __cplusplus
extern "C" {
#endif

enum {
    FZB_OK = 0,
    FZB_ERR_INVALID = 1,
    FZB_ERR_PANIC = 2,
    FZB_ERR_UNSUPPORTED = 3,
    FZB_ERR_HIP = 4,
    FZB_ERR_CAPACITY = 5
};

enum { FZB_CASE_IGNORE = 0, FZB_CASE_SMART = 1, FZB_CASE_RESPECT = 2 };
enum { FZB_UNICODE_IGNORE = 0, FZB_UNICODE_SMART = 1, FZB_UNICODE_ALWAYS = 2 };
enum { FZB_SORT_SCORE_THEN_INDEX_ASC = 0, FZB_SORT_SCORE_THEN_INDEX_DESC = 1, FZB_SORT_INDEX_ASC = 2, FZB_SORT_INDEX_DESC = 3 };
enum { FZB_MATCH_FUZZY = 0, FZB_MATCH_EXACT = 1, FZB_MATCH_PREFIX = 2, FZB_MATCH_SUFFIX = 3, FZB_MATCH_SUBSTRING = 4 };

typedef struct fzb_scoring {
    uint16_t match_score, mismatch_penalty, gap_open_penalty, gap_extend_penalty;
    uint16_t prefix_bonus, capitalization_bonus, matching_case_bonus, exact_match_bonus, delimiter_bonus;
} fzb_scoring;

typedef struct fzb_config {
    int32_t max_typos;
    int32_t casing;
    int32_t unicode;
    int32_t sort;
    fzb_scoring scoring;
    uint16_t pf_lanes, sw_lanes;
    int32_t matching;
} fzb_config;

typedef struct fzb_match {
    uint32_t index;
    uint16_t score;
    uint8_t exact;
    uint8_t _pad;
} fzb_match;

typedef struct fzb_matcher fzb_matcher;
typedef struct fzb_corpus fzb_corpus;

const char* fzb_last_error(void);

void fzb_config_default(fzb_config* out);

int fzb_matcher_create(const fzb_config* config, const uint8_t* needle_utf8, size_t needle_len, fzb_matcher** out);
int fzb_matcher_clone(const fzb_matcher* m, fzb_matcher** out);
int fzb_matcher_set_pattern(fzb_matcher* m, const uint8_t* needle_utf8, size_t needle_len);
int fzb_matcher_set_config(fzb_matcher* m, const fzb_config* config);
void fzb_matcher_free(fzb_matcher* m);
int fzb_matcher_info(const fzb_matcher* m, int32_t out[6]);

int fzb_corpus_upload(const uint8_t* bytes, const uint64_t* end_offsets, size_t n, fzb_corpus** out);
int fzb_corpus_from_device(const void* dev_bytes, const void* dev_ends, int ends_are_u64, size_t n, uint64_t total_bytes, fzb_corpus** out);
int fzb_corpus_set_max_len(fzb_corpus* c, uint32_t max_len);
int fzb_corpus_build_view(fzb_corpus* c, int* out_built);
int fzb_corpus_set_uniform_len(fzb_corpus* c, uint32_t len);
int fzb_corpus_signature_info(const fzb_corpus* c, int* out_built, uint64_t* out_bytes);
int fzb_corpus_signature_planes_info(const fzb_corpus* c, int* out_built, uint64_t* out_bytes);
void fzb_corpus_free(fzb_corpus* c);
size_t fzb_corpus_len(const fzb_corpus* c);

int fzb_corpus_reserve(fzb_corpus* c, size_t items, uint64_t bytes);
int fzb_corpus_append(fzb_corpus* c, const uint8_t* bytes, const uint64_t* end_offsets, size_t n_new);
int fzb_corpus_truncate(fzb_corpus* c, size_t n);
int fzb_corpus_info(const fzb_corpus* c, uint64_t out[12]);

int fzb_corpus_remove(fzb_corpus* c, const uint32_t* indices, size_t n_indices);
int fzb_corpus_remove_device(fzb_corpus* c, const void* dev_indices, size_t stride_bytes, const uint32_t* dev_count, size_t max_count);
int fzb_corpus_replace(fzb_corpus* c, const uint32_t* indices, size_t n, const uint8_t* bytes, const uint64_t* end_offsets);
int fzb_corpus_edit_info(const fzb_corpus* c, uint64_t out[4]);

int fzb_corpus_set_bias(fzb_corpus* c, const int16_t* values, size_t n);
int fzb_corpus_update_bias(fzb_corpus* c, const uint32_t* indices, const int16_t* values, size_t n);
int fzb_corpus_clear_bias(fzb_corpus* c);
int fzb_corpus_bias_info(const fzb_corpus* c, uint64_t out[4]);

int fzb_corpus_set_tags(fzb_corpus* c, const uint16_t* values, size_t n);
int fzb_corpus_update_tags(fzb_corpus* c, const uint32_t* indices, const uint16_t* values, size_t n);
int fzb_corpus_clear_tags(fzb_corpus* c);
int fzb_corpus_set_scope(fzb_corpus* c, uint16_t require, uint16_t exclude);
int fzb_corpus_scope_info(const fzb_corpus* c, uint64_t out[4]);

int fzb_match_list(fzb_matcher* m, const fzb_corpus* c, fzb_match** out, size_t* out_len);

int fzb_match_list_into(fzb_matcher* m, const fzb_corpus* c, size_t first, size_t count, uint32_t index_offset, fzb_match** out, size_t* out_len);

int fzb_matcher_reserve(fzb_matcher* m, const fzb_corpus* c);

int fzb_match_list_device(fzb_matcher* m, const fzb_corpus* c, size_t first, size_t count, uint32_t index_offset,
                          fzb_match* dev_out, size_t capacity, uint32_t* dev_count, void* stream);

int fzb_match_list_sorted_device(fzb_matcher* m, const fzb_corpus* c, fzb_match* dev_out, size_t capacity, uint32_t* dev_count, void* stream);

int fzb_match_list_top(fzb_matcher* m, const fzb_corpus* c, size_t limit, fzb_match** out, size_t* out_len, uint64_t* out_found);
int fzb_match_list_top_device(fzb_matcher* m, const fzb_corpus* c, size_t limit, fzb_match* dev_out, size_t capacity, uint32_t* dev_count, void* stream);

int fzb_match_list_parallel(fzb_matcher* m, const fzb_corpus* c, size_t threads, fzb_match** out, size_t* out_len);

void fzb_matches_free(fzb_match* p);

typedef struct fzb_sharded_corpus fzb_sharded_corpus;
enum {
    FZB_SHARD_BY_COUNT = 0,
    FZB_SHARD_BY_BYTES = 1,
    FZB_SHARD_OVERSUBSCRIBE = 2
};
int fzb_device_count(int* out);
int fzb_shard_ranges(const uint64_t* end_offsets, size_t n, int nshards, int by_bytes, uint64_t* out_bounds);
int fzb_corpus_upload_sharded(const uint8_t* bytes, const uint64_t* end_offsets, size_t n, int ndev, int flags, fzb_sharded_corpus** out);
void fzb_sharded_corpus_free(fzb_sharded_corpus* sc);
size_t fzb_sharded_corpus_len(const fzb_sharded_corpus* sc);
// ... 171 lines not shown
```

### include/frizbee_hip.hpp

```cpp
#pragma once
#include <cstdint>
#include <array>
#include <memory>
#include <optional>
#include <stdexcept>
#include <string>
#include <string_view>
#include <vector>

#include "frizbee_hip.h"

namespace frizbee {

struct Panic : std::runtime_error { using std::runtime_error::runtime_error; };
struct Error : std::runtime_error {
    int code;
    Error(int c, const std::string& m) : std::runtime_error(m), code(c) {}
};
inline void check(int rc) {
    if (rc == FZB_OK) return;
    const std::string msg = fzb_last_error();
    if (rc == FZB_ERR_PANIC) throw Panic(msg);
    throw Error(rc, msg);
}
// ... 96 lines not shown
        for (size_t i = 0; i < n; i++) {
            Pattern p(std::string((const char*)arr[i].needle_utf8, arr[i].needle_len));
            p.negated = arr[i].negated != 0;
            if (arr[i].matching >= 0) p.config.matching = (Matching)arr[i].matching;
            out.push_back(std::move(p));
        }
        fzb_patterns_free(arr, n);
        return out;
    }
};

class Corpus {
  public:
    template <typename Strings>
    explicit Corpus(const Strings& haystacks) {
        std::string bytes;
        std::vector<uint64_t> ends;
        for (const auto& h : haystacks) {
            const std::string_view v(h);
            bytes.append(v.data(), v.size());
            ends.push_back(bytes.size());
        }
        fzb_corpus* c = nullptr;
        check(fzb_corpus_upload((const uint8_t*)bytes.data(), ends.data(), ends.size(), &c));
        h_.reset(c);
    }
    size_t len() const { return fzb_corpus_len(h_.get()); }
    const fzb_corpus* raw() const { return h_.get(); }
    template <typename Strings>
    void append(const Strings& batch) {
        std::string bytes;
        std::vector<uint64_t> ends;
        for (const auto& h : batch) {
            const std::string_view v(h);
            bytes.append(v.data(), v.size());
            ends.push_back(bytes.size());
        }
        check(fzb_corpus_append(h_.get(), (const uint8_t*)bytes.data(), ends.data(), ends.size()));
    }
    void reserve(size_t items, uint64_t bytes) { check(fzb_corpus_reserve(h_.get(), items, bytes)); }
    void truncate(size_t n) { check(fzb_corpus_truncate(h_.get(), n)); }
    struct Info {
        uint64_t items, item_capacity, bytes, byte_capacity, max_len, uniform_len, has_view, view_nv, outliers, ends_u64, regrows, h2d_bytes;
    };
    Info info() const {
        uint64_t o[12] = {};
        check(fzb_corpus_info(h_.get(), o));
        return Info{o[0], o[1], o[2], o[3], o[4], o[5], o[6], o[7], o[8], o[9], o[10], o[11]};
    }
    uint64_t signature_planes_bytes() const {
        int built = 0;
        uint64_t bytes = 0;
        check(fzb_corpus_signature_planes_info(h_.get(), &built, &bytes));
        return built ? bytes : 0;
    }
    void remove(const std::vector<uint32_t>& indices) { check(fzb_corpus_remove(h_.get(), indices.data(), indices.size())); }
    void remove_device(const void* dev_indices, size_t stride_bytes, const uint32_t* dev_count, size_t max_count) {
        check(fzb_corpus_remove_device(h_.get(), dev_indices, stride_bytes, dev_count, max_count));
    }
    template <typename Strings>
    void replace(const std::vector<uint32_t>& indices, const Strings& batch) {
        std::string bytes;
        std::vector<uint64_t> ends;
        for (const auto& h : batch) {
            const std::string_view v(h);
            bytes.append(v.data(), v.size());
            ends.push_back(bytes.size());
        }
        if (ends.size() != indices.size()) throw Error(FZB_ERR_INVALID, "Corpus::replace: one haystack per index");
        check(fzb_corpus_replace(h_.get(), indices.data(), indices.size(), (const uint8_t*)bytes.data(), ends.data()));
    }
    struct EditInfo {
        uint64_t first, bytes_written, view_tiles, temp_bytes;
    };
    EditInfo edit_info() const {
        uint64_t o[4] = {};
        check(fzb_corpus_edit_info(h_.get(), o));
        return EditInfo{o[0], o[1], o[2], o[3]};
    }
    void set_bias(const std::vector<int16_t>& values) { check(fzb_corpus_set_bias(h_.get(), values.data(), values.size())); }
    void update_bias(const std::vector<uint32_t>& indices, const std::vector<int16_t>& values) {
        if (indices.size() != values.size()) throw Error(FZB_ERR_INVALID, "Corpus::update_bias: one value per index");
        check(fzb_corpus_update_bias(h_.get(), indices.data(), values.data(), indices.size()));
    }
    void clear_bias() { check(fzb_corpus_clear_bias(h_.get())); }
    struct BiasInfo {
        uint64_t has_bias, capacity, bias_hi, device_bytes;
    };
    BiasInfo bias_info() const {
        uint64_t o[4] = {};
        check(fzb_corpus_bias_info(h_.get(), o));
        return BiasInfo{o[0], o[1], o[2], o[3]};
    }
    void set_tags(const std::vector<uint16_t>& values) { check(fzb_corpus_set_tags(h_.get(), values.data(), values.size())); }
    void update_tags(const std::vector<uint32_t>& indices, const std::vector<uint16_t>& values) {
        if (indices.size() != values.size()) throw Error(FZB_ERR_INVALID, "Corpus::update_tags: one value per index");
        check(fzb_corpus_update_tags(h_.get(), indices.data(), values.data(), indices.size()));
    }
    void clear_tags() { check(fzb_corpus_clear_tags(h_.get())); }
    void set_scope(uint16_t require = 0, uint16_t exclude = 0) { check(fzb_corpus_set_scope(h_.get(), require, exclude)); }
    struct ScopeInfo {
        uint64_t active, capacity, scope, device_bytes;
        uint16_t require() const { return (uint16_t)(scope & 0xFFFF); }
        uint16_t exclude() const { return (uint16_t)(scope >> 16); }
    };
    ScopeInfo scope_info() const {
// ... 475 lines not shown
```

### rust/src/hip.rs

```rust
use crate::{CaseMatching, Config, Match, MatchIndices, Pattern, SortStrategy, UnicodeMatching};
use std::os::raw::{c_char, c_int, c_void};

#[repr(C)]
struct FzbScoring {
    match_score: u16,
    mismatch_penalty: u16,
    gap_open_penalty: u16,
    gap_extend_penalty: u16,
    prefix_bonus: u16,
    capitalization_bonus: u16,
    matching_case_bonus: u16,
    exact_match_bonus: u16,
    delimiter_bonus: u16,
}
#[repr(C)]
struct FzbConfig {
    max_typos: i32,
    casing: i32,
    unicode: i32,
    sort: i32,
    scoring: FzbScoring,
    pf_lanes: u16,
    sw_lanes: u16,
    matching: i32,
// ... 6 lines not shown
    exact: u8,
    _pad: u8,
}
#[repr(C)]
#[derive(Clone, Copy)]
#[allow(dead_code)]
struct FzbSection {
    require: u16,
    exclude: u16,
}
#[repr(C)]
#[derive(Clone, Copy)]
struct FzbMatchIndices {
    index: u32,
    score: u16,
    exact: u8,
    _pad: u8,
    positions_begin: u32,
    positions_len: u32,
}

#[repr(C)]
struct FzbPattern {
    needle_utf8: *const u8,
    needle_len: usize,
    negated: i32,
    has_max_typos: i32,
    max_typos: i32,
    casing: i32,
    unicode: i32,
    has_scoring: i32,
    scoring: FzbScoring,
    matching: i32,
}

const FZB_ERR_PANIC: c_int = 2;
const FZB_SHARD_BY_BYTES: c_int = 1;

#[link(name = "frizbee_hip")]
extern "C" {
    fn fzb_last_error() -> *const c_char;
    fn fzb_matcher_create(cfg: *const FzbConfig, needle: *const u8, len: usize, out: *mut *mut c_void) -> c_int;
    fn fzb_matcher_set_pattern(m: *mut c_void, needle: *const u8, len: usize) -> c_int;
    fn fzb_matcher_free(m: *mut c_void);
    fn fzb_corpus_upload(bytes: *const u8, ends: *const u64, n: usize, out: *mut *mut c_void) -> c_int;
    fn fzb_corpus_free(c: *mut c_void);
    fn fzb_corpus_append(c: *mut c_void, bytes: *const u8, ends: *const u64, n_new: usize) -> c_int;
    fn fzb_corpus_reserve(c: *mut c_void, items: usize, bytes: u64) -> c_int;
    fn fzb_corpus_truncate(c: *mut c_void, n: usize) -> c_int;
    #[allow(dead_code)]
    fn fzb_corpus_info(c: *const c_void, out: *mut u64) -> c_int;
    #[allow(dead_code)]
    fn fzb_corpus_signature_planes_info(c: *const c_void, out_built: *mut c_int, out_bytes: *mut u64) -> c_int;
    fn fzb_corpus_remove(c: *mut c_void, indices: *const u32, n_indices: usize) -> c_int;
    #[allow(dead_code)]
    fn fzb_corpus_remove_device(c: *mut c_void, dev_indices: *const c_void, stride_bytes: usize, dev_count: *const u32, max_count: usize) -> c_int;
    fn fzb_corpus_replace(c: *mut c_void, indices: *const u32, n: usize, bytes: *const u8, ends: *const u64) -> c_int;
    fn fzb_corpus_edit_info(c: *const c_void, out: *mut u64) -> c_int;
    fn fzb_corpus_set_bias(c: *mut c_void, values: *const i16, n: usize) -> c_int;
    fn fzb_corpus_update_bias(c: *mut c_void, indices: *const u32, values: *const i16, n: usize) -> c_int;
    fn fzb_corpus_clear_bias(c: *mut c_void) -> c_int;
    fn fzb_corpus_bias_info(c: *const c_void, out: *mut u64) -> c_int;
    fn fzb_corpus_set_tags(c: *mut c_void, values: *const u16, n: usize) -> c_int;
    fn fzb_corpus_update_tags(c: *mut c_void, indices: *const u32, values: *const u16, n: usize) -> c_int;
    fn fzb_corpus_clear_tags(c: *mut c_void) -> c_int;
    fn fzb_corpus_set_scope(c: *mut c_void, require: u16, exclude: u16) -> c_int;
    fn fzb_corpus_scope_info(c: *const c_void, out: *mut u64) -> c_int;
    fn fzb_corpus_len(c: *const c_void) -> usize;
    fn fzb_match_list(m: *mut c_void, c: *const c_void, out: *mut *mut FzbMatch, out_len: *mut usize) -> c_int;
    fn fzb_match_list_into(m: *mut c_void, c: *const c_void, first: usize, count: usize, index_offset: u32, out: *mut *mut FzbMatch, out_len: *mut usize) -> c_int;
    fn fzb_matches_free(p: *mut FzbMatch);
    fn fzb_match_list_top(m: *mut c_void, c: *const c_void, limit: usize, out: *mut *mut FzbMatch, out_len: *mut usize, out_found: *mut u64) -> c_int;
    #[allow(dead_code)]
    fn fzb_match_list_top_device(m: *mut c_void, c: *const c_void, limit: usize, dev_out: *mut FzbMatch, capacity: usize, dev_count: *mut u32, stream: *mut c_void) -> c_int;
    fn fzb_match_list_top_indices(m: *mut c_void, c: *const c_void, limit: usize, out: *mut *mut FzbMatchIndices, out_len: *mut usize, out_positions: *mut *mut u32,
                                  out_found: *mut u64) -> c_int;
    #[allow(dead_code)]
    fn fzb_match_list_top_indices_device(m: *mut c_void, c: *const c_void, limit: usize, dev_out: *mut FzbMatchIndices, capacity: usize, dev_positions: *mut u32,
                                         positions_capacity: usize, dev_count: *mut u32, stream: *mut c_void) -> c_int;
    fn fzb_matcher_reserve_top_indices(m: *mut c_void, c: *const c_void, limit: usize, max_needle_bytes: usize) -> c_int;
    fn fzb_corpus_generation(c: *const c_void, out: *mut u64) -> c_int;
    fn fzb_subset_create(c: *const c_void, out: *mut *mut c_void) -> c_int;
    fn fzb_subset_free(s: *mut c_void);
    fn fzb_subset_set_indices(s: *mut c_void, host_indices: *const u32, n: usize) -> c_int;
    fn fzb_subset_from_scope(s: *mut c_void, c: *const c_void, require: u16, exclude: u16) -> c_int;
    fn fzb_subset_info(s: *mut c_void, out: *mut u64) -> c_int;
    fn fzb_subset_read(s: *mut c_void, host_out: *mut u32, cap: usize, out_n: *mut usize) -> c_int;
    fn fzb_match_list_subset(m: *mut c_void, c: *const c_void, input: *const c_void, capture: *mut c_void, out: *mut *mut FzbMatch, out_len: *mut usize) -> c_int;
    fn fzb_match_list_top_subset(m: *mut c_void, c: *const c_void, input: *const c_void, capture: *mut c_void, limit: usize, out: *mut *mut FzbMatch, out_len: *mut usize,
                                 out_found: *mut u64) -> c_int;
    fn fzb_match_list_top_subset_device(m: *mut c_void, c: *const c_void, input: *const c_void, capture: *mut c_void, limit: usize, dev_out: *mut FzbMatch, capacity: usize,
                                        dev_count: *mut u32, stream: *mut c_void) -> c_int;
    fn fzb_match_list_top_indices_subset(m: *mut c_void, c: *const c_void, input: *const c_void, capture: *mut c_void, limit: usize, out: *mut *mut FzbMatchIndices,
                                         out_len: *mut usize, out_positions: *mut *mut u32, out_found: *mut u64) -> c_int;
    fn fzb_prompt_list_device(m: *mut c_void, c: *const c_void, input: *const c_void, first: usize, count: usize, index_offset: u32, dev_out: *mut FzbMatch, capacity: usize,
                              dev_count: *mut u32, stream: *mut c_void) -> c_int;
    fn fzb_prompt_top_device(m: *mut c_void, c: *const c_void, input: *const c_void, limit: usize, dev_out: *mut FzbMatch, capacity: usize, dev_count: *mut u32,
                             stream: *mut c_void) -> c_int;
    #[allow(dead_code)]
    fn fzb_facets_create(c: *const c_void, out: *mut *mut c_void) -> c_int;
    #[allow(dead_code)]
    fn fzb_facets_free(f: *mut c_void);
    #[allow(dead_code)]
    fn fzb_facets_read(f: *mut c_void, out: *mut u32) -> c_int;
    #[allow(dead_code)]
    fn fzb_facets_device(f: *const c_void) -> *const u32;
// ... 528 lines not shown
```

Before: 161.4 billion haystacks/s.

## Add repeat-letter signature planes to prefilter haystacks lacking needle's repeated letters

Builds a second bit-plane signature per haystack marking letter classes that occur at least twice, and computes a matching needle signature. The plane-based prefilter ANDs these extra planes into the candidate mask so haystacks missing the needle's repeated letters (e.g. 'deadbe' has two d's and e's) are rejected before the DFA stage. It also raises the number of in-flight plane loads per iteration from 4 to 8. The cost is an extra plane array in memory, a build kernel run at upload, and more plane reads per tile in the filter.

```diff
diff --git a/frizbee_amd/__init__.py b/frizbee_amd/__init__.py
--- a/frizbee_amd/__init__.py
+++ b/frizbee_amd/__init__.py
@@ -123,7 +123,7 @@
     "fzb_corpus_generation", "fzb_subset_create", "fzb_subset_free", "fzb_subset_set_indices", "fzb_subset_from_scope", "fzb_subset_info", "fzb_subset_read",
     "fzb_match_list_subset", "fzb_match_list_top_subset", "fzb_match_list_top_subset_device", "fzb_match_list_top_indices_subset",
     "fzb_multi_match_list_subset", "fzb_multi_match_list_top_subset", "fzb_multi_match_list_top_subset_device", "fzb_multi_match_list_top_indices_subset",
-    "fzb_debug_set_items_dfa_min", "fzb_debug_set_fused_capture", "fzb_debug_launch_grids", "fzb_corpus_signature_planes_info",
+    "fzb_debug_set_items_dfa_min", "fzb_debug_set_fused_capture", "fzb_debug_launch_grids", "fzb_corpus_signature_planes_info", "fzb_corpus_signature_repeat_planes_info",
     "fzb_prompt_list_device", "fzb_prompt_top_device",
     "fzb_facets_create", "fzb_facets_free", "fzb_facets_read", "fzb_facets_device", "fzb_matcher_set_facets", "fzb_multi_matcher_set_facets",
     "fzb_match_list_top_sections", "fzb_match_list_top_sections_device", "fzb_multi_match_list_top_sections", "fzb_multi_match_list_top_sections_device",
@@ -234,6 +234,7 @@
         l.fzb_multi_matcher_reserve_top_indices.argtypes = l.fzb_matcher_reserve_top_indices.argtypes
         l.fzb_corpus_signature_info.argtypes = [C.c_void_p, C.POINTER(C.c_int), C.POINTER(C.c_uint64)]
         l.fzb_corpus_signature_planes_info.argtypes = l.fzb_corpus_signature_info.argtypes
+        l.fzb_corpus_signature_repeat_planes_info.argtypes = l.fzb_corpus_signature_info.argtypes
         l.fzb_debug_needle_signature.argtypes = [C.c_void_p, C.POINTER(C.c_uint32), C.POINTER(C.c_int)]
         l.fzb_debug_signature_threshold.argtypes = []
         l.fzb_debug_signature_threshold.restype = C.c_uint32
@@ -425,7 +426,7 @@
                    "h2d_bytes")
     DEBUG_ARRAYS = {"bytes": (0, np.uint8), "ends": (1, None), "vbytes": (2, np.uint8), "vgofs": (3, np.uint32), "vgnv": (4, np.uint8), "vlen": (5, np.uint16),
                     "vperm": (6, np.uint16), "vlong": (7, np.uint32), "sig": (8, np.uint32), "bias": (9, np.int16), "tags": (10, np.uint16),
-                    "sig_planes": (11, np.uint64)}
+                    "sig_planes": (11, np.uint64), "sig_planes2": (12, np.uint64)}
 
     def set_bias(self, values):
         if values is None:
@@ -499,6 +500,11 @@
     def signature_planes_info(self):
         built, nbytes = C.c_int(), C.c_uint64()
         _check(lib().fzb_corpus_signature_planes_info(self.h, C.byref(built), C.byref(nbytes)))
+        return bool(built.value), int(nbytes.value)
+
+    def signature_repeat_planes_info(self):
+        built, nbytes = C.c_int(), C.c_uint64()
+        _check(lib().fzb_corpus_signature_repeat_planes_info(self.h, C.byref(built), C.byref(nbytes)))
         return bool(built.value), int(nbytes.value)
 
     def info(self):
diff --git a/frizbee_amd/csrc/fzb_internal.h b/frizbee_amd/csrc/fzb_internal.h
--- a/frizbee_amd/csrc/fzb_internal.h
+++ b/frizbee_amd/csrc/fzb_internal.h
@@ -68,6 +68,7 @@
     u32 n_long;
     const u32* sig;
     const u64* sig_planes;
+    const u64* sig_planes2;
 };
 
 struct fzb_match_rec {
@@ -175,9 +176,11 @@
                        u64* bitmap, u32* tile_counts, u32* reset_counters, int grid, hipStream_t st, u64* bitmap_m = nullptr, u32* tile_counts_m = nullptr,
                        u64* reject_bits = nullptr, u32* tile_rejects = nullptr, int nul_safe = 0, int acc_lo = -1, const u8* cdfa = nullptr, u32 cdfa_bytes = 0,
                        int cdfa_K = 0, int cdfa_G = 0, u32 needle_sig = 0, int sig_ok = 0,
-                       const SegList* seg = nullptr);
+                       const SegList* seg = nullptr,
+                       u32 needle_sig2 = 0);
 bool fzb_filter_sig_applies(const CorpusDev& c, int mode, u32 needle_sig, int sig_ok);
 void fzb_launch_sig_planes(const u32* sig, u64 n, u64 t0, u64* planes, int grid, hipStream_t st);
+void fzb_launch_sig_planes2(const CorpusDev& c, u64 n, u64 t0, u64* planes2, int grid, hipStream_t st);
 void fzb_launch_scan_rejects(const u32* tile_rejects, u32 ntiles, const u32* reject_count, u32* rej_prefix, hipStream_t st);
 void fzb_launch_init_counters(u32* counters, u32 n0, hipStream_t st);
 void fzb_launch_compact1(const u64* bitmap, const u32* counts, u32 n_items, const u32* n_items_ptr, const u32* src, u32* out_idx, u32* total_out, int grid, hipStream_t st,
diff --git a/frizbee_amd/csrc/host.hip b/frizbee_amd/csrc/host.hip
--- a/frizbee_amd/csrc/host.hip
+++ b/frizbee_amd/csrc/host.hip
@@ -816,6 +816,7 @@
     set_scorer_forms(m, needle_utf8, needle_len);
     m->sig_eligible = !m->unicode && lc.filter_mode == 1 && lc.filter_exact && needle_sig_eligible(needle_utf8, needle_len, k, m->literal_mode);
     m->needle_sig = m->sig_eligible ? needle_sig(needle_utf8, needle_len) : 0u;
+    m->needle_sig2 = m->sig_eligible ? needle_sig2(needle_utf8, needle_len) : 0u;
     return FZB_OK;
 }
 
@@ -987,6 +988,7 @@
     if (c->own_ends) (void)hipFree(c->own_ends);
     if (c->own_sig) (void)hipFree(c->own_sig);
     if (c->own_planes) (void)hipFree(c->own_planes);
+    if (c->own_planes2) (void)hipFree(c->own_planes2);
     fzb_column_release(c->bias);
     fzb_column_release(c->tags);
     if (c->pair_stage) (void)hipFree(c->pair_stage);
@@ -1620,7 +1622,7 @@
         p.segmented = true;
         FZB_PEV(2);
         fzb_launch_filter(p.cd, p.first, p.cnt, w.table, w.dfa, lc.dead_byte, nd.rows, 1, need, (u32)nd.min_haystack_len, w.bitmap, w.tile_counts, w.counters, (int)grid, p.st, nullptr, nullptr,
-                          nullptr, nullptr, lc.pad_ok, -1, nullptr, 0, 0, 0, m->needle_sig, 1, &p.seg);
+                          nullptr, nullptr, lc.pad_ok, -1, nullptr, 0, 0, 0, m->needle_sig, 1, &p.seg, m->needle_sig2);
         FZB_PEV(3);
         FZB_STAGE("filter(lists its survivors)");
         p.items = w.surv_idx;
diff --git a/frizbee_amd/csrc/host_internal.h b/frizbee_amd/csrc/host_internal.h
--- a/frizbee_amd/csrc/host_internal.h
+++ b/frizbee_amd/csrc/host_internal.h
@@ -57,6 +57,8 @@
     u64 sig_cap_items = 0;
     void* own_planes = nullptr;
     u64 planes_cap_tiles = 0;
+    void* own_planes2 = nullptr;
+    u64 planes2_cap_tiles = 0;
     int sig_device = -1;
     ItemColumn<int16_t> bias;
     u32 bias_hi = 0;
@@ -175,6 +177,7 @@
     std::vector<u8> cdfa;
     int cdfa_src = 0, cdfa_K = 0, cdfa_G = 0;
     u32 needle_sig = 0;
+    u32 needle_sig2 = 0;
     bool sig_eligible = false;
     bool long_needle = false;
     bool long_dfa = false;
diff --git a/frizbee_amd/csrc/host_upload.hip b/frizbee_amd/csrc/host_upload.hip
--- a/frizbee_amd/csrc/host_upload.hip
+++ b/frizbee_amd/csrc/host_upload.hip
@@ -596,25 +596,25 @@
     }
 }
 
-bool planes_ensure_room(fzb_corpus* c, u64 items, u64 keep_tiles) {
+bool planes_ensure_room(void*& own, u64& cap_tiles, const u64*& live, u64 items, u64 keep_tiles) {
     const u64 tiles = sig_plane_tiles(items);
-    if (c->own_planes && c->planes_cap_tiles >= tiles) return true;
+    if (own && cap_tiles >= tiles) return true;
     const size_t tile_bytes = 32 * FZB_SIG_PLANE_WORDS * sizeof(u64);
     void* p = nullptr;
     hipError_t e = fzb_dev_alloc(&p, (size_t)tiles * tile_bytes);
-    if (e == hipSuccess && keep_tiles && c->own_planes) e = hipMemcpy(p, c->own_planes, (size_t)std::min(keep_tiles, c->planes_cap_tiles) * tile_bytes, hipMemcpyDeviceToDevice);
-    if (c->own_planes) (void)hipFree(c->own_planes);
-    c->own_planes = nullptr;
-    c->planes_cap_tiles = 0;
+    if (e == hipSuccess && keep_tiles && own) e = hipMemcpy(p, own, (size_t)std::min(keep_tiles, cap_tiles) * tile_bytes, hipMemcpyDeviceToDevice);
+    if (own) (void)hipFree(own);
+    own = nullptr;
+    cap_tiles = 0;
     if (e != hipSuccess) {
         if (p) (void)hipFree(p);
         (void)hipGetLastError();
-        c->dev.sig_planes = nullptr;
+        live = nullptr;
         return false;
     }
-    c->own_planes = p;
-    c->planes_cap_tiles = tiles;
-    if (c->dev.sig_planes) c->dev.sig_planes = (const u64*)p;
+    own = p;
+    cap_tiles = tiles;
+    if (live) live = (const u64*)p;
     return true;
 }
 
@@ -625,12 +625,13 @@
     const bool want = !fzb_knobs().no_signature && n && c->dev.max_len != 0 && c->dev.max_len <= 32;
     if (!want) {
         c->dev.sig = nullptr;
-        c->dev.sig_planes = nullptr;
+        c->dev.sig_planes = c->dev.sig_planes2 = nullptr;
         return FZB_OK;
     }
-    if (!c->dev.sig) n_valid = 0, c->dev.sig_planes = nullptr;
+    if (!c->dev.sig) n_valid = 0, c->dev.sig_planes = c->dev.sig_planes2 = nullptr;
     n_valid = std::min(n_valid, n);
     const u64 planes_t0 = c->dev.sig_planes ? n_valid / FZB_SIG_PLANE_TILE : 0;
+    const u64 planes2_t0 = c->dev.sig_planes2 ? n_valid / FZB_SIG_PLANE_TILE : 0;
     if (!c->own_sig || c->sig_cap_items < n) {
         const u64 items = std::max<u64>(n, c->cap_items);
         void* p = nullptr;
@@ -640,7 +641,7 @@
             if (p) (void)hipFree(p);
             (void)hipGetLastError();
             c->dev.sig = nullptr;
-            c->dev.sig_planes = nullptr;
+            c->dev.sig_planes = c->dev.sig_planes2 = nullptr;
             if (e == hipErrorOutOfMemory) return FZB_OK;
             return fzb_fail(FZB_ERR_HIP, std::string("letter signatures: ") + hipGetErrorString(e));
         }
@@ -655,10 +656,15 @@
         else FZB_LAUNCH((k_sig_build<u32>), dim3(grid), dim3(UP_THREADS), 0, nullptr, c->dev.bytes, (const u32*)c->dev.ends, c->dev.uniform_len, n_valid, cnt, (u32*)c->own_sig);
     }
     c->dev.sig = (const u32*)c->own_sig;
-    if (planes_ensure_room(c, std::max<u64>(n, c->cap_items), planes_t0)) {
-        const u64 tiles = sig_plane_tiles(n);
+    const u64 tiles = sig_plane_tiles(n);
+    if (planes_ensure_room(c->own_planes, c->planes_cap_tiles, c->dev.sig_planes, std::max<u64>(n, c->cap_items), planes_t0)) {
         if (planes_t0 < tiles) fzb_launch_sig_planes(c->dev.sig, n, planes_t0, (u64*)c->own_planes, (int)fzb_grid_cap(tiles - planes_t0, 8), nullptr);
         c->dev.sig_planes = (const u64*)c->own_planes;
+    }
+    if (!c->dev.sig_planes) c->dev.sig_planes2 = nullptr;
+    else if (planes_ensure_room(c->own_planes2, c->planes2_cap_tiles, c->dev.sig_planes2, std::max<u64>(n, c->cap_items), planes2_t0)) {
+        if (planes2_t0 < tiles) fzb_launch_sig_planes2(c->dev, n, planes2_t0, (u64*)c->own_planes2, (int)fzb_grid_cap(tiles - planes2_t0, 8), nullptr);
+        c->dev.sig_planes2 = (const u64*)c->own_planes2;
     }
     return FZB_OK;
 }
@@ -680,9 +686,11 @@
         c->own_sig = nullptr; c->sig_cap_items = 0;
         if (c->own_planes) (void)hipFree(c->own_planes);
         c->own_planes = nullptr; c->planes_cap_tiles = 0;
+        if (c->own_planes2) (void)hipFree(c->own_planes2);
+        c->own_planes2 = nullptr; c->planes2_cap_tiles = 0;
     }
     c->dev.sig = nullptr;
-    c->dev.sig_planes = nullptr;
+    c->dev.sig_planes = c->dev.sig_planes2 = nullptr;
     if (!fzb_knobs().verify_promises) return FZB_OK;
     HIPCHK(hipDeviceSynchronize());
     const int rc = fzb_sig_sync(c, 0);
@@ -1127,8 +1135,11 @@
             (void)hipGetLastError();
         }
     }
-    if (!fzb_knobs().no_signature && (!c->dev.n || (c->dev.max_len != 0 && c->dev.max_len <= 32)) && c->own_sig && c->sig_cap_items >= c->cap_items)
-        (void)planes_ensure_room(c, c->cap_items, c->dev.sig_planes ? sig_plane_tiles(c->dev.n) : 0);
+    if (!fzb_knobs().no_signature && (!c->dev.n || (c->dev.max_len != 0 && c->dev.max_len <= 32)) && c->own_sig && c->sig_cap_items >= c->cap_items) {
+        if (planes_ensure_room(c->own_planes, c->planes_cap_tiles, c->dev.sig_planes, c->cap_items, c->dev.sig_planes ? sig_plane_tiles(c->dev.n) : 0))
+            (void)planes_ensure_room(c->own_planes2, c->planes2_cap_tiles, c->dev.sig_planes2, c->cap_items, c->dev.sig_planes2 ? sig_plane_tiles(c->dev.n) : 0);
+        if (!c->dev.sig_planes) c->dev.sig_planes2 = nullptr;
+    }
     HIPCHK(hipDeviceSynchronize());
     return FZB_OK;
 }
@@ -1239,6 +1250,13 @@
     return FZB_OK;
 }
 
+int fzb_corpus_signature_repeat_planes_info(const fzb_corpus* c, int* out_built, uint64_t* out_bytes) {
+    if (!c) return fzb_fail(FZB_ERR_INVALID, "null argument");
+    if (out_built) *out_built = c->dev.sig_planes2 != nullptr;
+    if (out_bytes) *out_bytes = c->dev.sig_planes2 ? sig_plane_words(c->dev.n) * 8 : 0;
+    return FZB_OK;
+}
+
 int fzb_debug_corpus_read(const fzb_corpus* c, int what, void* host_out, size_t cap_bytes, size_t* out_bytes) {
     if (!c || !out_bytes) return fzb_fail(FZB_ERR_INVALID, "null argument");
     const u64 n = c->dev.n, groups = up_tiles(n) * (UP_TILE / 64);
@@ -1258,6 +1276,7 @@
         case 9: src = c->bias.data; bytes = c->bias.live ? (size_t)n * sizeof(int16_t) : 0; break;
         case 10: src = c->tags.data; bytes = c->tags.live ? (size_t)n * sizeof(uint16_t) : 0; break;
         case 11: src = c->dev.sig_planes; bytes = c->dev.sig_planes ? (size_t)sig_plane_words(n) * 8 : 0; break;
+        case 12: src = c->dev.sig_planes2; bytes = c->dev.sig_planes2 ? (size_t)sig_plane_words(n) * 8 : 0; break;
         default: return fzb_fail(FZB_ERR_INVALID, "fzb_debug_corpus_read: unknown array " + std::to_string(what));
     }
     *out_bytes = bytes;
diff --git a/frizbee_amd/csrc/kernels_filter.hip b/frizbee_amd/csrc/kernels_filter.hip
--- a/frizbee_amd/csrc/kernels_filter.hip
+++ b/frizbee_amd/csrc/kernels_filter.hip
@@ -228,8 +228,11 @@
     return total;
 }
 
+#ifndef FZB_SIG_CAND_INFLIGHT
+#define FZB_SIG_CAND_INFLIGHT 8
+#endif
 template <typename ET>
-__device__ __forceinline__ void sig_planes_run(const u8* __restrict__ bytes, const ET* __restrict__ ends, const u64* __restrict__ planes, u32 nsig, u64 first, u32 count, u32 rows,
+__device__ __forceinline__ void sig_planes_run(const u8* __restrict__ bytes, const ET* __restrict__ ends, const u64* __restrict__ planes, u32 nsig, const u64* __restrict__ planes2, u32 nsig2, u64 first, u32 count, u32 rows,
                                                u32 min_len, u32 acc_lo, u64* __restrict__ bitmap, u32* __restrict__ tile_counts, u32 ulen, u32 gather_max, const SegList& seg, u8* dfa, const u8* __restrict__ dfa_g) {
     constexpr u32 B = FZB_SIG_BATCH_TILES;
     static_assert(B * 16 <= 256 && B * 32 <= 256 && B * FZB_TILE <= 65536, "a batch's words are one per thread, its positions fit the queue's u16");
@@ -245,22 +248,26 @@
     tc_run(ntiles, seg.stride / FZB_TILE, blockIdx.x, &t_begin, &t_end);
     u32* const seg_out = seg.list + (size_t)blockIdx.x * seg.stride;
     const u32 j = tid >> 4, w = tid & 15u;
+    const u64 need = (u64)nsig | ((u64)nsig2 << 32);
+    const ptrdiff_t to2 = nsig2 ? (ptrdiff_t)((uintptr_t)planes2 - (uintptr_t)planes) : 0;
     auto load_cand = [&](u32 tb, u32 nb) -> u64 {
         if (tid >= nb * 16) return 0;
         u64 cand = sig_plane_valid(tb + j, w, count);
-        const u64* pl = planes + sig_plane_index(tile0 + tb + j, 0, w);
-        u32 m = nsig;
+        const u8* pl = (const u8*)(planes + sig_plane_index(tile0 + tb + j, 0, w));
+        u64 m = need;
         while (m) {
-            u64 v[4];
-#pragma unroll
-            for (int q = 0; q < 4; q++) {
+            u64 v[FZB_SIG_CAND_INFLIGHT];
+#pragma unroll
+            for (int q = 0; q < FZB_SIG_CAND_INFLIGHT; q++) {
                 v[q] = ~0ull;
                 if (m) {
-                    v[q] = pl[(u32)__builtin_ctz(m) * FZB_SIG_PLANE_WORDS];
+                    const u32 k = (u32)__builtin_ctzll(m);
+                    v[q] = *(const u64*)(pl + (k < 32u ? (ptrdiff_t)(k * FZB_SIG_PLANE_WORDS * 8u) : to2 + (ptrdiff_t)((k - 32u) * FZB_SIG_PLANE_WORDS * 8u)));
                     m &= m - 1u;
                 }
             }
-            cand &= (v[0] & v[1]) & (v[2] & v[3]);
+#pragma unroll
+            for (int q = 0; q < FZB_SIG_CAND_INFLIGHT; q++) cand &= v[q];
         }
         return cand;
     };
@@ -355,13 +362,13 @@
 template <typename ET, bool SEG, bool PLANES = false>
 __global__ __launch_bounds__(256) __attribute__((amdgpu_waves_per_eu(8, 8))) void k1_dfa_sig(const u8* __restrict__ bytes, const ET* __restrict__ ends, const u32* __restrict__ sig, u32 nsig, u64 first, u32 count,
                                                   const u8* __restrict__ dfa_g, int rows, u32 min_len, u32 acc_lo, u64* __restrict__ bitmap, u32* __restrict__ tile_counts,
-                                                  u32* __restrict__ reset_counters, u32 ulen, u32 gather_max, SegList seg) {
+                                                  u32* __restrict__ reset_counters, u32 ulen, u32 gather_max, SegList seg, const u64* __restrict__ planes2, u32 nsig2) {
     if (blockIdx.x == 0 && threadIdx.x < 16) reset_counters[threadIdx.x] = 0;
     extern __shared__ __attribute__((aligned(16))) u8 dfa[];
     if constexpr (PLANES) {
         static_assert(SEG, "the plane form lists its survivors");
         dfa_require_lds_base0(dfa);
-        sig_planes_run<ET>(bytes, ends, (const u64*)sig, nsig, first, count, (u32)rows, min_len, acc_lo, bitmap, tile_counts, ulen, gather_max, seg, dfa, dfa_g);
+        sig_planes_run<ET>(bytes, ends, (const u64*)sig, nsig, planes2, nsig2, first, count, (u32)rows, min_len, acc_lo, bitmap, tile_counts, ulen, gather_max, seg, dfa, dfa_g);
         return;
     }
     u32& s_cnt = *(u32*)(dfa + FZB_DFA_LDS_BYTES(rows));
@@ -1014,32 +1021,73 @@
 #undef FZB_K1I
 }
 
+__device__ __forceinline__ void sig_planes_put(u32 s, u32 p, u64* s_pl) {
+    const u32 tid = threadIdx.x, lane = tid & 63, wave = tid >> 6;
+    u64 mine = 0;
+    for (u32 b = 0; b < 32; b++) {
+        const u64 bal = __ballot((s >> b) & 1u);
+        if (lane == b) mine = bal;
+    }
+    if (lane < 32) s_pl[lane * FZB_SIG_PLANE_WORDS + p * 4 + wave] = mine;
+}
+__device__ __forceinline__ void sig_planes_store(const u64* s_pl, u64* __restrict__ planes, u64 tile) {
+    const u32 tid = threadIdx.x;
+    __syncthreads();
+    u64* out = planes + sig_plane_index(tile, 0, 0);
+    out[tid] = s_pl[tid];
+    out[tid + 256] = s_pl[tid + 256];
+    __syncthreads();
+}
 __global__ __launch_bounds__(256) void k_sig_planes_build(const u32* __restrict__ sig, u64 n, u64 t0, u64* __restrict__ planes) {
     __shared__ u64 s_pl[32 * FZB_SIG_PLANE_WORDS];
-    const u32 tid = threadIdx.x, lane = tid & 63, wave = tid >> 6;
     const u64 tiles = sig_plane_tiles(n);
     for (u64 tile = t0 + blockIdx.x; tile < tiles; tile += gridDim.x) {
 #pragma unroll
         for (u32 p = 0; p < FZB_TILE / 256; p++) {
-            const u64 i = tile * FZB_TILE + p * 256 + tid;
-            const u32 s = i < n ? sig[i] : 0u;
-            u64 mine = 0;
-            for (u32 b = 0; b < 32; b++) {
-                const u64 bal = __ballot((s >> b) & 1u);
-                if (lane == b) mine = bal;
-            }
-            if (lane < 32) s_pl[lane * FZB_SIG_PLANE_WORDS + p * 4 + wave] = mine;
-        }
-        __syncthreads();
-        u64* out = planes + sig_plane_index(tile, 0, 0);
-        out[tid] = s_pl[tid];
-        out[tid + 256] = s_pl[tid + 256];
-        __syncthreads();
+            const u64 i = tile * FZB_TILE + p * 256 + threadIdx.x;
+            sig_planes_put(i < n ? sig[i] : 0u, p, s_pl);
+        }
+        sig_planes_store(s_pl, planes, tile);
     }
 }
 void fzb_launch_sig_planes(const u32* sig, u64 n, u64 t0, u64* planes, int grid, hipStream_t st) {
     FZB_LAUNCH(k_sig_planes_build, dim3(std::max(1, grid)), dim3(256), 0, st, sig, n, t0, planes);
 }
+template <typename ET>
+__global__ __launch_bounds__(256) void k_sig_planes2_build(const u8* __restrict__ bytes, const ET* __restrict__ ends, u32 ulen, u64 n, u64 t0, u64* __restrict__ planes2) {
+    __shared__ u64 s_pl[32 * FZB_SIG_PLANE_WORDS];
+    const u64 tiles = sig_plane_tiles(n);
+    for (u64 tile = t0 + blockIdx.x; tile < tiles; tile += gridDim.x) {
+#pragma unroll
+        for (u32 p = 0; p < FZB_TILE / 256; p++) {
+            const u64 i = tile * FZB_TILE + p * 256 + threadIdx.x;
+            u32 once = 0, s = 0;
+            if (i < n) {
+                u64 hs;
+                u32 L;
+                haystack_span_u(ends, ulen, i, hs, L);
+                L = min(L, 32u);
+                const uint4* vp = (const uint4*)(bytes + hs);
+                uint4 a = make_uint4(0, 0, 0, 0), b = make_uint4(0, 0, 0, 0);
+                if (L > 0) a = vp[0];
+                if (L > 16) b = vp[1];
+                u32 w[8] = {a.x, a.y, a.z, a.w, b.x, b.y, b.z, b.w};
+#pragma unroll
+                for (int q = 0; q < 8; q++) {
+                    const u32 nvb = L > 4u * q ? L - 4u * q : 0u;
+                    if (nvb < 4) w[q] &= (1u << (8 * nvb)) - 1;
+                    sig2_accum_word(w[q], once, s);
+                }
+            }
+            sig_planes_put(s, p, s_pl);
+        }
+        sig_planes_store(s_pl, planes2, tile);
+    }
+}
+void fzb_launch_sig_planes2(const CorpusDev& c, u64 n, u64 t0, u64* planes2, int grid, hipStream_t st) {
+    if (c.ends_u64) FZB_LAUNCH((k_sig_planes2_build<u64>), dim3(std::max(1, grid)), dim3(256), 0, st, c.bytes, (const u64*)c.ends, c.uniform_len, n, t0, planes2);
+    else FZB_LAUNCH((k_sig_planes2_build<u32>), dim3(std::max(1, grid)), dim3(256), 0, st, c.bytes, (const u32*)c.ends, c.uniform_len, n, t0, planes2);
+}
 
 bool fzb_filter_sig_applies(const CorpusDev& c, int mode, u32 needle_sig, int sig_ok) {
     return mode == 1 && c.max_len != 0 && c.max_len <= 32 && sig_ok && needle_sig && c.sig && !fzb_knobs().no_signature;
@@ -1047,7 +1095,7 @@
 
 void fzb_launch_filter(const CorpusDev& c, u64 first, u32 count, const u64* table, const u8* dfa, u32 dead, int rows, int mode, int need, u32 min_len,
                        u64* bitmap, u32* tile_counts, u32* reset_counters, int grid, hipStream_t st, u64* bitmap_m, u32* tile_counts_m, u64* reject_bits, u32* tile_rejects, int nul_safe,
-                       int acc_lo, const u8* cdfa, u32 cdfa_bytes, int cdfa_K, int cdfa_G, u32 needle_sig, int sig_ok, const SegList* seg) {
+                       int acc_lo, const u8* cdfa, u32 cdfa_bytes, int cdfa_K, int cdfa_G, u32 needle_sig, int sig_ok, const SegList* seg, u32 needle_sig2) {
     const u32 acc = acc_lo < 0 ? (u32)rows : (u32)acc_lo;
     const u32 ntiles = (count + FZB_TILE - 1) / FZB_TILE;
     const int cus = std::max(1, grid / 8);
@@ -1060,9 +1108,11 @@
             const u32 gmax = std::min<u32>(FZB_SIG_GATHER_MAX, FZB_TILE);
             const bool planes = seg && c.sig_planes && first % FZB_TILE == 0 && !fzb_knobs().no_sig_planes;
             const size_t lds_s = planes ? FZB_DFA_LDS_BYTES(rows) + FZB_SIG_BATCH_TILES * (4 + 256 + 2 * (size_t)gmax) : lds + 128 + 2 * FZB_TILE;
-#define FZB_K1S(ET, SEG, PL, G, S) FZB_LAUNCH((k1_dfa_sig<ET, SEG, PL>), dim3(G), dim3(256), lds_s, st, c.bytes, (const ET*)c.ends, PL ? (const u32*)c.sig_planes : c.sig, needle_sig, first, count, dfa, rows, min_len, acc, bitmap, tile_counts, reset_counters, c.uniform_len, gmax, S)
+#define FZB_K1S(ET, SEG, PL, G, S) FZB_LAUNCH((k1_dfa_sig<ET, SEG, PL>), dim3(G), dim3(256), lds_s, st, c.bytes, (const ET*)c.ends, PL ? (const u32*)c.sig_planes : c.sig, needle_sig, first, count, dfa, rows, min_len, acc, bitmap, tile_counts, reset_counters, c.uniform_len, gmax, S, PL ? c.sig_planes2 : nullptr, PL ? nsig2 : 0u)
+            const u32 nsig2 = planes && c.sig_planes2 ? needle_sig2 : 0u;
             if (planes) {
                 if (g_fzb_record_grids) fzb_record_grid("k1_dfa_sig_planes", seg->nseg);
+                if (g_fzb_record_grids && nsig2) fzb_record_grid("k1_dfa_sig_repeat", seg->nseg);
                 if (c.ends_u64) FZB_K1S(u64, true, true, seg->nseg, *seg); else FZB_K1S(u32, true, true, seg->nseg, *seg);
             } else if (seg) {
                 if (c.ends_u64) FZB_K1S(u64, true, false, seg->nseg, *seg); else FZB_K1S(u32, true, false, seg->nseg, *seg);
diff --git a/frizbee_amd/csrc/sig_filter.h b/frizbee_amd/csrc/sig_filter.h
--- a/frizbee_amd/csrc/sig_filter.h
+++ b/frizbee_amd/csrc/sig_filter.h
@@ -48,6 +48,31 @@
     for (uint32_t m = nsig; m; m &= m - 1u) c &= planes[sig_plane_index(tile, (uint32_t)__builtin_ctz(m), word)];
     return c;
 }
+FZB_SIG_FN void sig2_accum_byte(uint32_t b, uint32_t& once, uint32_t& twice) {
+    const uint32_t s = sig_of_byte(b);
+    twice |= once & s;
+    once |= s;
+}
+FZB_SIG_FN void sig2_accum_word(uint32_t w, uint32_t& once, uint32_t& twice) {
+    sig2_accum_byte(w & 0xFF, once, twice);
+    sig2_accum_byte((w >> 8) & 0xFF, once, twice);
+    sig2_accum_byte((w >> 16) & 0xFF, once, twice);
+    sig2_accum_byte(w >> 24, once, twice);
+}
+FZB_SIG_FN uint32_t sig2_of_bytes(const uint8_t* p, size_t n) {
+    uint32_t once = 0, twice = 0;
+    for (size_t i = 0; i < n; i++) sig2_accum_byte(p[i], once, twice);
+    return twice;
+}
+FZB_SIG_FN uint32_t needle_sig2(const uint8_t* needle, size_t n) { return sig2_of_bytes(needle, n); }
+FZB_SIG_FN bool sig2_passes(uint32_t sig, uint32_t sig2, uint32_t nsig, uint32_t nsig2) { return sig_passes(sig, nsig) && (sig2 & nsig2) == nsig2; }
+FZB_SIG_FN void sig_planes2_transpose_ref(const uint32_t* sig2, uint64_t n, uint64_t* planes2) { sig_planes_transpose_ref(sig2, n, planes2); }
+FZB_SIG_FN uint64_t sig_plane_candidates2(const uint64_t* planes, const uint64_t* planes2, uint64_t tile, uint32_t word, uint32_t nsig, uint32_t nsig2) {
+    uint64_t c = sig_plane_candidates(planes, tile, word, nsig);
+    for (uint32_t m = nsig2; m; m &= m - 1u) c &= planes2[sig_plane_index(tile, (uint32_t)__builtin_ctz(m), word)];
+    return c;
+}
+
 #ifndef FZB_SIG_BATCH_TILES
 #define FZB_SIG_BATCH_TILES 8u
 #endif
diff --git a/include/frizbee_hip.h b/include/frizbee_hip.h
--- a/include/frizbee_hip.h
+++ b/include/frizbee_hip.h
@@ -65,6 +65,7 @@
 int fzb_corpus_set_uniform_len(fzb_corpus* c, uint32_t len);
 int fzb_corpus_signature_info(const fzb_corpus* c, int* out_built, uint64_t* out_bytes);
 int fzb_corpus_signature_planes_info(const fzb_corpus* c, int* out_built, uint64_t* out_bytes);
+int fzb_corpus_signature_repeat_planes_info(const fzb_corpus* c, int* out_built, uint64_t* out_bytes);
 void fzb_corpus_free(fzb_corpus* c);
 size_t fzb_corpus_len(const fzb_corpus* c);
 
diff --git a/include/frizbee_hip.hpp b/include/frizbee_hip.hpp
--- a/include/frizbee_hip.hpp
+++ b/include/frizbee_hip.hpp
@@ -172,6 +172,12 @@
         int built = 0;
         uint64_t bytes = 0;
         check(fzb_corpus_signature_planes_info(h_.get(), &built, &bytes));
+        return built ? bytes : 0;
+    }
+    uint64_t signature_repeat_planes_bytes() const {
+        int built = 0;
+        uint64_t bytes = 0;
+        check(fzb_corpus_signature_repeat_planes_info(h_.get(), &built, &bytes));
         return built ? bytes : 0;
     }
     void remove(const std::vector<uint32_t>& indices) { check(fzb_corpus_remove(h_.get(), indices.data(), indices.size())); }
diff --git a/rust/src/hip.rs b/rust/src/hip.rs
--- a/rust/src/hip.rs
+++ b/rust/src/hip.rs
@@ -82,6 +82,8 @@
     fn fzb_corpus_info(c: *const c_void, out: *mut u64) -> c_int;
     #[allow(dead_code)]
     fn fzb_corpus_signature_planes_info(c: *const c_void, out_built: *mut c_int, out_bytes: *mut u64) -> c_int;
+    #[allow(dead_code)]
+    fn fzb_corpus_signature_repeat_planes_info(c: *const c_void, out_built: *mut c_int, out_bytes: *mut u64) -> c_int;
     fn fzb_corpus_remove(c: *mut c_void, indices: *const u32, n_indices: usize) -> c_int;
     #[allow(dead_code)]
     fn fzb_corpus_remove_device(c: *mut c_void, dev_indices: *const c_void, stride_bytes: usize, dev_count: *const u32, max_count: usize) -> c_int;
```

After: 172.1 billion haystacks/s (median of 6 runs). +6.6%, better.
